# damemi/odigos

Measured on AMD Instinct MI355X. Metric: spans/sec processed (whole node) at 1/2/4/8 MI355X; % of HBM roofline, higher is better.
Workload: dtype u8; 1 GPU; C4: fused odigossampling -> odigosurltemplate -> odigostrafficmetrics, 100M spans in total (all on one GPU at N=1; ~100M/N per GPU, trace-id all-to-all over RCCL at N>1); spans_per_gpu=100000000, spans_total=100000000, template_form=refs, seed=219545604, parallelism=dp1: independent span shards, no data-path collective

## Files before the change

odigos_amd/csrc/engine.cpp:

```cpp
#include <hip/hip_runtime.h>

#include <algorithm>
#include <map>
#include <cstdio>
#include <cstdlib>
#include <cstring>
#include <mutex>
#include <string>
#include <unordered_map>
#include <vector>

#include "../../include/odigos_amd.h"
#include "config.hpp"
#include "devcfg.hpp"
#include "engine_internal.hpp"
#include "kernels.hpp"
#include "slab.hpp"

namespace ose {

thread_local std::string g_last_error;

int fail(int code, const std::string& msg) {
  g_last_error = msg;
  return code;
}

Engine::~Engine() {
  release_exchange_scratch(this);
  release_batch_pool(this);
  release_otlp(this);
  release_encode(this);
  release_condattr(this);
  for (auto& t : timings) { (void)hipEventDestroy(t.a); (void)hipEventDestroy(t.b); }
  for (auto s : streams) (void)hipStreamDestroy(s);
  for (auto ev : event_pool) (void)hipEventDestroy(ev);
  if (url_blob_dev) (void)hipFree(url_blob_dev);
  if (url_blob_forced_dev) (void)hipFree(url_blob_forced_dev);
  for (auto* d : sampling_chunks_dev)
    if (d) (void)hipFree(d);
  for (auto* d : sampling_svc_map_dev)
    if (d) (void)hipFree(d);
  if (sampling_svc_maps_dev) (void)hipFree(sampling_svc_maps_dev);
  if (shard_tables_dev) (void)hipFree(shard_tables_dev);
  if (path_count_dev) (void)hipFree(path_count_dev);
  if (attr_blob_dev) (void)hipFree(attr_blob_dev);
  if (attr_host_mask_dev) (void)hipFree(attr_host_mask_dev);
  for (auto* w : pool) delete w;
}

Workspace::~Workspace() {
  if (dev) (void)hipFree(dev);
  if (table) (void)hipFree(table);
  if (dup_bkt) (void)hipFree(dup_bkt);
  if (dup_bkt_count) (void)hipFree(dup_bkt_count);
  if (runs) (void)hipFree(runs);
  if (run_count) (void)hipFree(run_count);
  if (attr_bits) (void)hipFree(attr_bits);
  if (ep_planes) (void)hipFree(ep_planes);
  if (svc_local) (void)hipFree(svc_local);
  for (void* f : fold)
    if (f) (void)hipFree(f);
  if (dup_host) (void)hipHostFree(dup_host);
  for (hipEvent_t ev : {pending, dup_ready, fork, join, join2})
    if (ev) (void)hipEventDestroy(ev);
}

hipEvent_t Engine::take_event() {
  if (!event_pool.empty()) {
    hipEvent_t ev = event_pool.back();
    event_pool.pop_back();
    return ev;
  }
  hipEvent_t ev = nullptr;
  (void)hipEventCreate(&ev);
  return ev;
}
Engine::Timed Engine::prof_begin(const char* name, hipStream_t st) {
  std::lock_guard<std::mutex> g(mu);
  Timed t{name, take_event(), take_event()};
  (void)hipEventRecord(t.a, st);
  return t;
}
void Engine::prof_end(Timed& t, hipStream_t st) {
  (void)hipEventRecord(t.b, st);
  std::lock_guard<std::mutex> g(mu);
  timings.push_back(t);
}
void Engine::prof_drop(Timed& t) {
  std::lock_guard<std::mutex> g(mu);
  event_pool.push_back(t.a);
  event_pool.push_back(t.b);
}
int Engine::launch_status() {
  HIP_TRY(hipGetLastError());
  return 0;
}

bool stream_capturing(hipStream_t st) {
  hipStreamCaptureStatus cs = hipStreamCaptureStatusNone;
  return hipStreamIsCapturing(st, &cs) == hipSuccess && cs != hipStreamCaptureStatusNone;
}

Workspace* Engine::acquire_ws(hipStream_t st) {
  if (stream_capturing(st)) {
    std::lock_guard<std::mutex> g(mu);
    Workspace* w = nullptr;
    if (!free_ws.empty()) {
      auto it = std::max_element(free_ws.begin(), free_ws.end(),
                                 [](const Workspace* a, const Workspace* b) { return a->cap < b->cap; });
      w = *it;
      free_ws.erase(it);
    } else {
      w = new Workspace();
      pool.push_back(w);
    }
    w->captured = true;
    return w;
  }
  Workspace* w = nullptr;
  {
    std::lock_guard<std::mutex> g(mu);
    if (!free_ws.empty()) {
      w = free_ws.back();
      free_ws.pop_back();
    } else {
      w = new Workspace();
      pool.push_back(w);
    }
  }
  if (w->pending_set) (void)hipStreamWaitEvent(st, w->pending, 0);
  return w;
}
void Engine::return_unused_ws(Workspace* w) {
  std::lock_guard<std::mutex> g(mu);
  w->captured = false;
  free_ws.push_back(w);
}
void Engine::release_ws(Workspace* w, hipStream_t st) {
  if (w->captured) return;
  if (!w->pending) (void)hipEventCreateWithFlags(&w->pending, hipEventDisableTiming);
  w->pending_set = w->pending && hipEventRecord(w->pending, st) == hipSuccess;
  std::lock_guard<std::mutex> g(mu);
  free_ws.push_back(w);
}
#ifndef OSE_SIDE_STREAM_PRIO
#define OSE_SIDE_STREAM_PRIO 0
#endif
hipStream_t Engine::take_stream() {
  std::lock_guard<std::mutex> g(mu);
  if (!free_streams.empty()) {
    hipStream_t s = free_streams.back();
    free_streams.pop_back();
    return s;
  }
  hipStream_t s = nullptr;
#if OSE_SIDE_STREAM_PRIO
  int least = 0, greatest = 0;
  (void)hipDeviceGetStreamPriorityRange(&least, &greatest);
  if (hipStreamCreateWithPriority(&s, hipStreamNonBlocking, greatest) != hipSuccess) return nullptr;
#else
  if (hipStreamCreateWithFlags(&s, hipStreamNonBlocking) != hipSuccess) return nullptr;
#endif
  streams.push_back(s);
  return s;
}
void Engine::give_stream(hipStream_t s) {
  std::lock_guard<std::mutex> g(mu);
  free_streams.push_back(s);
}

int Workspace::reserve(size_t bytes) {
  if (bytes <= cap) return 0;
  if (captured) return fail(OSE_ENOMEM, "workspace too small inside a hipGraph capture: call ose_reserve first");
  if (dev) HIP_TRY(hipFree(dev));
  dev = nullptr;
  cap = 0;
  size_t want = std::max<size_t>(bytes, 1 << 20);
  HIP_TRY(hipMalloc(&dev, want));
  cap = want;
  return 0;
}

int ensure_device() {
  static int status = 1;
  static std::mutex m;
  std::lock_guard<std::mutex> g(m);
  if (status == 1) {
    int n = 0;
    hipError_t e = hipGetDeviceCount(&n);
    status = (e == hipSuccess && n > 0) ? 0 : OSE_EDEVICE;
  }
  if (status) return fail(OSE_EDEVICE, "no HIP device visible: the odigos_amd engine runs only on an MI355X (gfx950)");
  return 0;
}

int bind_device(const Engine* e) {
  int cur = -1;
  if (hipGetDevice(&cur) != hipSuccess || cur != e->device) HIP_TRY(hipSetDevice(e->device));
  return 0;
}

static std::mutex g_dropped_mu;
static uint64_t g_dropped_count = 0;
static std::string g_dropped_last;
void note_dropped_error(const char* where, hipError_t err) {
  std::lock_guard<std::mutex> g(g_dropped_mu);
  g_dropped_count++;
  g_dropped_last = std::string(where) + ": " + hipGetErrorName(err) + " (" + hipGetErrorString(err) + ")";
}

void engine_retain(Engine* e) { e->refs.fetch_add(1, std::memory_order_relaxed); }

void engine_unref(Engine* e) {
  if (e->refs.fetch_sub(1, std::memory_order_acq_rel) != 1) return;
  LastErrorScope keep("engine_unref");
  (void)bind_device(e);
  (void)hipDeviceSynchronize();
  delete e;
}

int upload(const std::vector<uint8_t>& host, uint8_t** dev) {
  HIP_TRY(hipMalloc(dev, host.size()));
  HIP_TRY(hipMemcpy(*dev, host.data(), host.size(), hipMemcpyHostToDevice));
  return 0;
}

int download_columns(const ose_columns& c, const ose_columns* dst) {
  const uint64_t n = c.n_spans, R = c.n_resources, S = c.n_scopes, K = c.n_attr_keys;
  struct F { const void* src; void* dst; size_t bytes; };
  const F fs[] = {
      {c.arena, (void*)dst->arena, c.arena_bytes}, {c.trace_id, (void*)dst->trace_id, 16 * n},
      {c.start_ns, (void*)dst->start_ns, 8 * n}, {c.end_ns, (void*)dst->end_ns, 8 * n},
      {c.status, (void*)dst->status, n}, {c.kind, (void*)dst->kind, n}, {c.resource, (void*)dst->resource, 4 * n},
      {c.scope, (void*)dst->scope, 4 * n}, {c.url_flags, (void*)dst->url_flags, n}, {c.path, (void*)dst->path, 8 * n},
      {c.route, (void*)dst->route, 8 * n}, {c.span_size, (void*)dst->span_size, 4 * n},
      {c.name_len, (void*)dst->name_len, 4 * n},
      {c.attr_match, (void*)dst->attr_match, 8 * n * std::max<uint32_t>(1, c.attr_match_words)},
      {c.res_svc, (void*)dst->res_svc, 4 * R}, {c.res_svc_str, (void*)dst->res_svc_str, 4 * R},
      {c.res_url_ok, (void*)dst->res_url_ok, R}, {c.res_attrset, (void*)dst->res_attrset, 4 * R},
      {c.res_size, (void*)dst->res_size, 4 * R}, {c.scope_size, (void*)dst->scope_size, 4 * S},
      {c.scope_resource, (void*)dst->scope_resource, 4 * S}, {c.attr_type, (void*)dst->attr_type, K * n},
      {c.attr_val, (void*)dst->attr_val, 8 * K * n}, {c.db_flags, (void*)dst->db_flags, n},
      {c.db_query, (void*)dst->db_query, 8 * n}, {c.res_sql_ok, (void*)dst->res_sql_ok, R},
  };
  for (auto& f : fs)
    if (f.src && f.dst && f.bytes) HIP_TRY(hipMemcpy(f.dst, f.src, f.bytes, hipMemcpyDefault));
  return 0;
}

namespace {
int check_stage_mask(const Engine* e, const ose_columns* c, const ose_outputs* o, uint32_t mask) {
  if (mask & OSE_STAGE_CONDATTR) return refuse_condattr("ose_process and ose_process_device");
  if (mask & ~(OSE_STAGE_SAMPLE | OSE_STAGE_TEMPLATE | OSE_STAGE_SIZE | OSE_STAGE_APPLY_KEEP | OSE_STAGE_TEMPLATE_REFS |
               OSE_STAGE_APPLY_TEMPLATE | OSE_STAGE_SQLOP | OSE_STAGE_APPLY_SQLOP))
    return fail(OSE_EINVAL, "unknown stage bit");
  if ((mask & OSE_STAGE_TEMPLATE_REFS) && !(mask & OSE_STAGE_TEMPLATE))
    return fail(OSE_EINVAL, "OSE_STAGE_TEMPLATE_REFS needs OSE_STAGE_TEMPLATE");
  if ((mask & OSE_STAGE_APPLY_KEEP) && (mask & OSE_STAGE_SAMPLE))
    return fail(OSE_EINVAL, "OSE_STAGE_APPLY_KEEP and OSE_STAGE_SAMPLE exclude each other");
  if ((mask & OSE_STAGE_APPLY_TEMPLATE) && (mask & OSE_STAGE_TEMPLATE))
    return fail(OSE_EINVAL, "OSE_STAGE_APPLY_TEMPLATE and OSE_STAGE_TEMPLATE exclude each other");
  if ((mask & OSE_STAGE_APPLY_SQLOP) && (mask & OSE_STAGE_SQLOP))
    return fail(OSE_EINVAL, "OSE_STAGE_APPLY_SQLOP and OSE_STAGE_SQLOP exclude each other");
  if (mask & OSE_STAGE_SQLOP) {
    if (!e->has_sqlop) return fail(OSE_EINVAL, "odigossqldboperationprocessor is not configured on this engine");
    if (!c->db_flags || !c->db_query || !c->resource || !o->sql_op)
      return fail(OSE_EINVAL, "SQLOP stage needs db_flags, db_query, resource and sql_op");
  }
  return 0;
}

struct UrlFork {
  Engine* e;
  Workspace* ws;
  hipStream_t st;
  hipStream_t ust = nullptr;
  bool early_join = false;
  bool join_recorded = false;
  void open() {
    if (!ws->fork) (void)hipEventCreateWithFlags(&ws->fork, hipEventDisableTiming);
    if (!ws->join) (void)hipEventCreateWithFlags(&ws->join, hipEventDisableTiming);
    if (!ws->join2) (void)hipEventCreateWithFlags(&ws->join2, hipEventDisableTiming);
    if (ws->fork && ws->join && ws->join2) ust = e->take_stream();
    if (ust && (hipEventRecord(ws->fork, st) != hipSuccess || hipStreamWaitEvent(ust, ws->fork, 0) != hipSuccess)) {
      e->give_stream(ust);
      ust = nullptr;
    }
  }
  void join(hipEvent_t ev, bool recorded, int& rc) {
    const hipError_t je = recorded ? hipSuccess : hipEventRecord(ev, ust);
    const hipError_t jw = je == hipSuccess ? hipStreamWaitEvent(st, ev, 0) : je;
    if (jw != hipSuccess) {
      (void)hipStreamSynchronize(ust);
      if (!rc) rc = fail(OSE_EDEVICE, std::string("URL stream join: ") + hipGetErrorString(jw));
    }
  }
  void close() {
    if (ust) e->give_stream(ust);
    ust = nullptr;
  }
};

void fuse_size_into_copy(UrlKernelArgs& ua, SizeKernelArgs& sa, Workspace* ws, size_t size_off, const ose_columns* c) {
  sa.kept_partials = size_partials_of(ws, size_off, c->n_scopes, c->n_resources);
  sa.n_kept_partials = url_copy_blocks(ua.n_groups);
  ua.fuse_size = 1;
  ua.size_partials = const_cast<uint32_t*>(sa.kept_partials);
  ua.sz = sa;
}
}

StageOffsets stage_offsets(uint32_t mask, bool defer, uint64_t n, uint64_t n_scopes, uint64_t n_resources,
                           uint64_t arena_bytes, uint32_t url_words) {
  const bool sample = mask & OSE_STAGE_SAMPLE;
  StageOffsets s{};
  s.need = sample ? sampling_scratch_bytes(n) : 0;
  s.url_off = sample ? up(defer ? s.need : 256) : 0;
  s.size_off = sample ? 256 : 0;
  if (mask & OSE_STAGE_TEMPLATE) {
    const size_t url_end = s.url_off + url_workspace_bytes(n, arena_bytes, url_words);
    s.need = std::max(s.need, url_end);
    s.size_off = up(url_end);
  }
  if (mask & OSE_STAGE_SIZE) s.need = std::max(s.need, s.size_off + size_scratch_bytes(n_scopes, n_resources));
  return s;
}

size_t Engine::workspace_bytes(uint64_t n_spans, uint64_t arena_bytes) const {
  const uint32_t mask = (has_sampling ? OSE_STAGE_SAMPLE : 0) | (has_url ? OSE_STAGE_TEMPLATE : 0) |
                        (has_traffic ? OSE_STAGE_SIZE : 0);
  if (has_sampling && has_traffic && !has_url) return sampling_scratch_bytes(n_spans) + size_scratch_bytes(n_spans, n_spans);
  return up(stage_offsets(mask, true, n_spans, n_spans, n_spans, arena_bytes, url_words()).need);
}

int run_stages(Engine* e, const ose_columns* c, const ose_outputs* o, uint32_t mask, uint32_t group_mode,
               const ose_rand* rnd, hipStream_t st) {
  if (!c || !o) return fail(OSE_EINVAL, "columns and outputs are required");
  if (const int mrc = check_stage_mask(e, c, o, mask)) return mrc;
  const bool sql_size = (mask & OSE_STAGE_SIZE) && (mask & (OSE_STAGE_SQLOP | OSE_STAGE_APPLY_SQLOP));
  if (sql_size)
    if (const int src = check_sqlop_size(c, o)) return src;
  const bool capturing = stream_capturing(st);
  if (capturing && (mask & OSE_STAGE_SAMPLE) && group_mode == OSE_GROUP_TRACE_ID)
    return fail(OSE_ENOTSUP, "SAMPLE with OSE_GROUP_TRACE_ID cannot be captured into a hipGraph "
                             "(its trace-id tables advance a host-side generation per call)");
  Workspace* ws = e->acquire_ws(st);
  const uint64_t n = c->n_spans;
  const bool gate_on_host = (mask & OSE_STAGE_SAMPLE) && group_mode == OSE_GROUP_TRACE_ID && n > 0 && !capturing &&
                            !(OSE_DIAG && getenv("OSE_NO_DEFER_SLOW"));
  const bool defer = gate_on_host && (mask & OSE_STAGE_TEMPLATE);
  const StageOffsets so = stage_offsets(mask, defer, n, c->n_scopes, c->n_resources, c->arena_bytes, e->url_words());
  int rc = ws->reserve(so.need);
  const bool tmpl = !rc && (mask & OSE_STAGE_TEMPLATE);
  const bool fused_size_ok = !sql_size && !(OSE_DIAG && getenv("OSE_NO_FUSED_SIZE"));
  std::function<int()> sample_tail;
  UrlKernelArgs ua{};
  UrlFork fork{e, ws, st};
  static const bool one_stream = getenv("OSE_ONE_STREAM") != nullptr;
  constexpr uint64_t kForkSpans = 1u << 20;
  if (!one_stream && !rc && defer && n >= kForkSpans) fork.open();
  ws->beside_url = fork.ust && tmpl;
#ifndef OSE_URL_JOIN_LATE
  fork.early_join = fork.ust && tmpl && (mask & OSE_STAGE_TEMPLATE_REFS) && (mask & OSE_STAGE_SIZE) && fused_size_ok;
#endif
  const uint32_t plan_groups = (uint32_t)((n + kUrlGroup - 1) / kUrlGroup);
  UrlRun ur;
  ur.ws_off = so.url_off;
  ur.refs = (mask & OSE_STAGE_TEMPLATE_REFS) != 0;
  ur.grid_mult = url_plan_grid_mult(plan_groups, fork.ust != nullptr);
  ur.planned = fork.early_join ? ws->join : nullptr;
  if (fork.ust && tmpl) {
    rc = run_url(e, c, o, fork.ust, ws, ur, &ua);
    fork.join_recorded = fork.early_join && !rc;
  }
  if (!rc && (mask & OSE_STAGE_SAMPLE)) rc = run_sampling(e, c, o, group_mode, rnd, st, ws, gate_on_host ? &sample_tail : nullptr);
  if (sample_tail && !defer) {
    rc = sample_tail();
    sample_tail = nullptr;
  }
  if (!fork.ust && tmpl && !rc) rc = run_url(e, c, o, st, ws, ur, &ua);
  if (sample_tail) {
    const int trc = sample_tail();
    if (!rc) rc = trc;
  }
  if (fork.ust) fork.join(ws->join, fork.join_recorded, rc);
  if (!rc && (mask & OSE_STAGE_SQLOP)) rc = run_sqlop(e, c, o, st);
  SizeKernelArgs sa{};
  bool size_on = false;
  if (!rc && (mask & OSE_STAGE_SIZE)) rc = prepare_size(e, c, o, mask, group_mode, rnd, st, ws, so.size_off, sa, size_on);
  if (!rc && tmpl) {
    if (size_on && n > 0 && fused_size_ok) fuse_size_into_copy(ua, sa, ws, so.size_off, c);
    rc = run_url_back(e, ua, st);
  }
  if (!rc && size_on) rc = sql_size ? run_sqlop_size_tail(e, sa, o->sql_op, st) : run_size_tail(e, sa, st);
  if (fork.join_recorded) fork.join(ws->join2, false, rc);
  fork.close();
  ws->beside_url = false;
  e->release_ws(ws, st);
  return rc;
}

}

using namespace ose;

extern "C" {

const char* ose_last_error(void) { return g_last_error.c_str(); }

uint64_t ose_dropped_errors(char* last, size_t cap) {
  std::lock_guard<std::mutex> g(g_dropped_mu);
  if (last && cap) snprintf(last, cap, "%s", g_dropped_last.c_str());
  return g_dropped_count;
}

extern "C" void osehost_stage_offsets(uint32_t mask, int defer, uint64_t n_spans, uint64_t n_scopes, uint64_t n_resources,
                                      uint64_t arena_bytes, uint32_t url_words, uint64_t* out) {
  const StageOffsets so = stage_offsets(mask, defer != 0, n_spans, n_scopes, n_resources, arena_bytes, url_words);
  Engine e;
  e.has_sampling = mask & OSE_STAGE_SAMPLE;
  e.has_url = mask & OSE_STAGE_TEMPLATE;
  e.has_traffic = mask & OSE_STAGE_SIZE;
  e.url_nfa_words = url_words;
  out[0] = so.url_off;
  out[1] = so.size_off;
  out[2] = so.need;
  out[3] = e.workspace_bytes(n_spans, arena_bytes);
}

int ose_engine_create(const char* cfg_json, ose_engine** out) {
  if (!out) return fail(OSE_EINVAL, "out is NULL");
  *out = nullptr;
  Json root;
  try {
    root = parse_json(cfg_json ? cfg_json : "{}");
  } catch (const std::exception& ex) {
    return fail(OSE_EINVAL, ex.what());
  }
  if (!root.is_obj()) return fail(OSE_EINVAL, "config must be a JSON object");
  auto* e = new Engine();
  std::string err;
  if (const Json* j = root.get("odigosurltemplate")) {
    err = decode_url_config(*j, e->url);
    if (!err.empty()) { delete e; return fail(OSE_EINVAL, err); }
    e->has_url = true;
    e->url_needs_resource = e->url.include.has_value() || e->url.exclude.has_value();
  }
  if (const Json* j = root.get("odigossampling")) {
    err = decode_sampling_config(*j, e->sampling);
    if (!err.empty()) { delete e; return fail(OSE_EINVAL, err); }
    e->has_sampling = true;
  }
  if (const Json* j = root.get("odigostrafficmetrics")) {
    err = decode_traffic_config(*j, e->traffic);
    if (!err.empty()) { delete e; return fail(OSE_EINVAL, err); }
    e->has_traffic = true;
    e->inverse = e->traffic.sampling_ratio != 0 ? (int64_t)(1.0 / e->traffic.sampling_ratio) : 0;
  }
  if (const Json* j = root.get("odigossqldboperationprocessor")) {
    err = decode_sqlop_config(*j, e->sqlop);
    if (!err.empty()) { delete e; return fail(OSE_EINVAL, err); }
    e->has_sqlop = true;
  }
  if (const Json* j = root.get("odigosconditionalattributes")) {
    err = decode_condattr_config(*j, e->condattr);
    if (!err.empty()) { delete e; return fail(OSE_EINVAL, err); }
    if (const int crc = compile_condattr(e->condattr, e->condattr_tab)) { delete e; return crc; }
    e->has_condattr = true;
  }
  if (e->has_url) {
    int rc = build_url_blob(e->url, e->url_blob_host, e->max_name, false, e->url_nfa_words);
    if (rc) { delete e; return rc; }
  }
  int rc = e->build_sampling_tables();
  if (rc) { delete e; return rc; }
  rc = e->build_attr_tables();
  if (rc) { delete e; return rc; }
  rc = ensure_device();
  if (rc) { delete e; return rc; }
  if (hipGetDevice(&e->device) != hipSuccess) { delete e; return fail(OSE_EDEVICE, "hipGetDevice failed"); }
  if (e->has_url) {
    rc = upload(e->url_blob_host, &e->url_blob_dev);
    if (rc) { delete e; return rc; }
  }
  rc = e->upload_sampling_tables();
  if (rc) { delete e; return rc; }
  if (e->has_condattr) {
    rc = upload(e->condattr_tab.blob, &e->condattr_blob_dev);
    if (rc) { delete e; return rc; }
  }
  if (!e->attr_blob_host.empty()) {
    rc = upload(e->attr_blob_host, &e->attr_blob_dev);
    if (rc) { delete e; return rc; }
    std::vector<uint8_t> hm(8 * std::max<size_t>(e->attr_words, 1), 0);
    std::memcpy(hm.data(), e->attr_host_words.data(), 8 * std::min<size_t>(e->attr_host_words.size(), e->attr_words));
    rc = upload(hm, &e->attr_host_mask_dev);
    if (rc) { delete e; return rc; }
  }
  {
    hipError_t he = hipMalloc(reinterpret_cast<void**>(&e->path_count_dev), 64);
    if (he == hipSuccess) he = hipMemset(e->path_count_dev, 0, 64);
    if (he != hipSuccess) {
      delete e;
      return fail(OSE_EDEVICE, std::string("path counters: ") + hipGetErrorString(he));
    }
  }
  *out = reinterpret_cast<ose_engine*>(e);
  return 0;
}

uint32_t ose_engine_path_counts(ose_engine* eng, uint64_t* counts, uint32_t cap) {
  if (!eng) return 0;
  Engine* e = reinterpret_cast<Engine*>(eng);
  uint64_t c[5] = {0, 0, 0, 0, 0};
  if (e->path_count_dev && bind_device(e) == 0) {
    LastErrorScope keep("ose_engine_path_counts");
    if (hipDeviceSynchronize() != hipSuccess ||
        hipMemcpy(c, e->path_count_dev, 32, hipMemcpyDeviceToHost) != hipSuccess)
      c[0] = c[1] = c[2] = c[3] = 0;
  }
  c[4] = c[3];
  c[3] = c[2];
  c[2] = e->long_run_passes.load();
  for (uint32_t k = 0; k < 5 && k < cap && counts; k++) counts[k] = c[k];
  return 5;
}

uint64_t ose_engine_url_nfa_groups(ose_engine* eng) {
  if (!eng) return 0;
  Engine* e = reinterpret_cast<Engine*>(eng);
  uint64_t c = 0;
  if (e->path_count_dev && bind_device(e) == 0) {
    LastErrorScope keep("ose_engine_url_nfa_groups");
    if (hipDeviceSynchronize() != hipSuccess || hipMemcpy(&c, e->path_count_dev + 4, 8, hipMemcpyDeviceToHost) != hipSuccess)
      c = 0;
  }
  return c;
}

void ose_engine_destroy(ose_engine* eng) {
  if (!eng) return;
  Engine* e = reinterpret_cast<Engine*>(eng);
  e->closed.store(true);
  engine_unref(e);
}

int ose_host_alloc(size_t bytes, void** out) {
  if (!out) return fail(OSE_EINVAL, "NULL argument");
  int rc = ensure_device();
  if (rc) return rc;
  HIP_TRY(hipHostMalloc(out, bytes ? bytes : 1, hipHostMallocDefault));
  return 0;
}
void ose_host_free(void* p) {
  LastErrorScope keep("ose_host_free");
  if (p) (void)hipHostFree(p);
}

int ose_set_device(int device) {
  int rc = ensure_device();
  if (rc) return rc;
  HIP_TRY(hipSetDevice(device));
  return 0;
}

uint32_t ose_engine_service_id(const ose_engine* eng, const char* name, size_t len) {
  if (!eng || !name) return OSE_NONE;
  const Engine* e = reinterpret_cast<const Engine*>(eng);
  auto it = e->service_ids.find(std::string(name, len));
  return it == e->service_ids.end() ? OSE_NONE : it->second;
}

int ose_engine_get_info(const ose_engine* eng, ose_engine_info* info) {
  if (!eng || !info) return fail(OSE_EINVAL, "NULL argument");
  const Engine* e = reinterpret_cast<const Engine*>(eng);
  info->stages = (e->has_sampling ? OSE_STAGE_SAMPLE : 0) | (e->has_url ? OSE_STAGE_TEMPLATE : 0) |
                 (e->has_traffic ? OSE_STAGE_SIZE : 0) | (e->has_sqlop ? OSE_STAGE_SQLOP : 0) |
                 (e->has_condattr ? OSE_STAGE_CONDATTR : 0);
  info->max_template_name = e->max_name;
  info->inverse_sampling = e->inverse;
  info->traffic_sampling_ratio = e->traffic.sampling_ratio;
  info->n_attr_rules = e->attr_n_rules;
  info->n_attr_keys = (uint32_t)e->attr_keys.size();
  info->attr_host_rules = e->attr_host_rules;
  return 0;
}

uint32_t ose_engine_attr_host_rules(const ose_engine* eng, uint64_t* words, uint32_t cap) {
  if (!eng) return 0;
  const Engine* e = reinterpret_cast<const Engine*>(eng);
  if (!e->attr_n_rules) return 0;
  const uint32_t W = e->attr_words;
  for (uint32_t w = 0; w < W && w < cap && words; w++) words[w] = w < e->attr_host_words.size() ? e->attr_host_words[w] : 0;
  return W;
}

int ose_engine_set_option(ose_engine* eng, const char* name, int64_t value) {
  if (!eng || !name) return fail(OSE_EINVAL, "NULL argument");
  Engine* e = reinterpret_cast<Engine*>(eng);
  static const struct { const char* name; uint32_t bit; } kOpts[] = {
      {"otlp_gpu_chain", Engine::kOptOtlpGpuChain},
      {"otlp_host_resources", Engine::kOptOtlpHostResources},
      {"otlp_host_scopes", Engine::kOptOtlpHostScopes},
      {"encode_host", Engine::kOptEncodeHost},
      {"otlp_sqlop", Engine::kOptOtlpSqlop},
      {"url_path_counts", Engine::kOptUrlPathCounts},
      {"otlp_condattr", Engine::kOptOtlpCondattr},
      {"url_regex_nfa", Engine::kOptUrlRegexNfa},
  };
  for (const auto& o : kOpts) {
    if (strcmp(name, o.name) != 0) continue;
    if (o.bit == Engine::kOptOtlpSqlop && !e->has_sqlop)
      return fail(OSE_EINVAL, "engine option otlp_sqlop: odigossqldboperationprocessor is not configured");
    if (o.bit == Engine::kOptOtlpCondattr) {
      if (!e->has_condattr)
        return fail(OSE_EINVAL, "engine option otlp_condattr: odigosconditionalattributes is not configured");
      if (value)
        if (const int rc = build_condattr_keytab(e)) return rc;
    }
    if (o.bit == Engine::kOptUrlRegexNfa) {
      if (!e->has_url) return fail(OSE_EINVAL, "engine option url_regex_nfa: odigosurltemplate is not configured");
      if (value && !e->url_blob_forced_dev) {
        if (int brc = bind_device(e)) return brc;
        std::vector<uint8_t> blob;
        uint32_t max_name = 0, words = 0;
        if (const int rc = build_url_blob(e->url, blob, max_name, true, words)) return rc;
        if (const int rc = upload(blob, &e->url_blob_forced_dev)) return rc;
        e->url_forced_words = words;
      }
    }
    if (value) e->options.fetch_or(o.bit);
    else e->options.fetch_and(~o.bit);
    return 0;
  }
  return fail(OSE_EINVAL, std::string("unknown engine option: ") + name);
}

int ose_reserve(ose_engine* eng, uint64_t n_spans, uint64_t arena_bytes) {
  if (!eng) return fail(OSE_EINVAL, "NULL engine");
  Engine* e = reinterpret_cast<Engine*>(eng);
  if (int brc = bind_device(e)) return brc;
  Workspace* ws = e->acquire_ws(nullptr);
  int rc = ws->reserve(e->workspace_bytes(n_spans, arena_bytes));
  if (!rc && e->has_sampling) rc = ws->reserve_table(n_spans);
  if (!rc && e->attr_n_dev) rc = ws->reserve_attr(n_spans);
  if (!rc && e->sampling_chunks_dev.size() > 1) rc = ws->reserve_fold(std::max<uint64_t>(n_spans, 1));
  e->release_ws(ws, nullptr);
  return rc;
}

int ose_process_device(ose_engine* eng, const ose_columns* cols, const ose_outputs* outs, uint32_t stage_mask,
                       uint32_t group_mode, const ose_rand* rnd, void* hip_stream) {
  if (!eng) return fail(OSE_EINVAL, "NULL engine");
  if (int brc = bind_device(reinterpret_cast<Engine*>(eng))) return brc;
  return run_stages(reinterpret_cast<Engine*>(eng), cols, outs, stage_mask, group_mode, rnd,
                    static_cast<hipStream_t>(hip_stream));
}

int ose_profile_enable(ose_engine* eng, int on) {
  if (!eng) return fail(OSE_EINVAL, "NULL engine");
  reinterpret_cast<Engine*>(eng)->profiling = on != 0;
  return 0;
}

int ose_profile_read(ose_engine* eng, char* json, size_t cap) {
  if (!eng || !json) return fail(OSE_EINVAL, "NULL argument");
  Engine* e = reinterpret_cast<Engine*>(eng);
  if (int brc = bind_device(e)) return brc;
  std::vector<Engine::Timed> ts;
  {
    std::lock_guard<std::mutex> g(e->mu);
    ts.swap(e->timings);
  }
  std::map<std::string, std::pair<uint64_t, double>> acc;
  for (auto& t : ts) {
    HIP_TRY(hipEventSynchronize(t.b));
    float ms = 0;
    HIP_TRY(hipEventElapsedTime(&ms, t.a, t.b));
    auto& a = acc[t.name];
    a.first++;
    a.second += ms;
  }
  {
    std::lock_guard<std::mutex> g(e->mu);
    for (auto& t : ts) { e->event_pool.push_back(t.a); e->event_pool.push_back(t.b); }
  }
  std::string s = "{";
  for (auto& kv : acc) {
    if (s.size() > 1) s += ",";
    char buf[256];
    snprintf(buf, sizeof buf, "\"%s\":{\"launches\":%llu,\"ms\":%.6f}", kv.first.c_str(),
             (unsigned long long)kv.second.first, kv.second.second);
    s += buf;
  }
  s += "}";
  if (s.size() + 1 > cap) return fail(OSE_ERANGE, "profile buffer too small");
  std::memcpy(json, s.c_str(), s.size() + 1);
  return 0;
}

int ose_device_info(char* buf, size_t cap) {
  if (!buf || cap == 0) return fail(OSE_EINVAL, "NULL buffer");
  int rc = ensure_device();
  if (rc) { snprintf(buf, cap, "no device"); return rc; }
  hipDeviceProp_t p;
  HIP_TRY(hipGetDeviceProperties(&p, 0));
  snprintf(buf, cap, "%s arch=%s CUs=%d HBM=%.1fGB", p.name, p.gcnArchName, p.multiProcessorCount,
           (double)p.totalGlobalMem / 1e9);
  return 0;
}

}
```

odigos_amd/csrc/engine_internal.hpp:

```cpp
#pragma once
#include <hip/hip_runtime.h>

#include <atomic>
#include <cstdint>
#include <functional>
#include <mutex>
#include <string>
#include <unordered_map>
#include <vector>

#include "../../include/odigos_amd.h"
#include "config.hpp"
#include "condattr_host.hpp"
#include "slab.hpp"
#include "timed_launch.hpp"

namespace ose {

int fail(int code, const std::string& msg);
#define HIP_TRY(expr)                                                                                  \
  do {                                                                                                 \
    hipError_t _e = (expr);                                                                            \
    if (_e != hipSuccess) return fail(OSE_EDEVICE, std::string(#expr) + ": " + hipGetErrorString(_e)); \
  } while (0)
struct Engine;
int bind_device(const Engine* e);
int upload(const std::vector<uint8_t>& host, uint8_t** dev);
int ensure_device();
void engine_retain(Engine* e);
void engine_unref(Engine* e);
void note_dropped_error(const char* where, hipError_t err);
struct LastErrorScope {
  const char* where;
  hipError_t prev;
  explicit LastErrorScope(const char* w) : where(w), prev(hipPeekAtLastError()) {}
  ~LastErrorScope() {
    if (prev != hipSuccess) return;
    const hipError_t now = hipGetLastError();
    if (now != hipSuccess) note_dropped_error(where, now);
  }
};
bool stream_capturing(hipStream_t st);
struct Engine;
void release_exchange_scratch(const Engine* e);
void release_batch_pool(Engine* e);
struct OtlpEngine;
void release_otlp(Engine* e);
void release_encode(Engine* e);
void release_condattr(Engine* e);
int build_condattr_keytab(Engine* e);

struct OtlpBatchView {
  Engine* e;
  const ose_columns* cols;
  bool released;
  const uint64_t* d_spans;
  bool res_on_device;
  const uint64_t *d_res_ref, *d_scope_ref;
  const uint64_t *h_res_ref, *h_scope_ref;
  size_t h_res_n, h_scope_n;
};
void otlp_batch_view(const ose_otlp_batch* b, OtlpBatchView* v);
struct OtlpReleasedLayout {
  const uint64_t* spans;
  const uint32_t* span0;
  const uint64_t *hdr, *schema;
  const uint64_t* res_ref;
  const uint32_t* res_scope0;
  const uint64_t* scope_ref;
};
ose_otlp_batch* otlp_released_new(Engine* e);
void otlp_released_delete(ose_otlp_batch* b);
int otlp_released_arena(ose_otlp_batch* b, size_t bytes, uint8_t** p);
void otlp_released_set(ose_otlp_batch* b, const ose_columns& cols, const OtlpReleasedLayout& lay);

struct Workspace {
  void* dev = nullptr;
  size_t cap = 0;
  hipEvent_t pending = nullptr;
  bool pending_set = false;
  bool captured = false;
  int reserve(size_t bytes);
  void* table = nullptr;
  uint64_t table_slots_cap = 0;
  uint64_t* dup_bkt = nullptr;
  uint32_t* dup_bkt_count = nullptr;
  uint32_t dup_bkt_bits = 0;
  uint32_t epoch = 0;
  int reserve_table(uint64_t n_spans);
  uint32_t* runs = nullptr;
  uint32_t* run_count = nullptr;
  uint64_t runs_slots = 0;
  int reserve_runs();
  void* fold[2] = {nullptr, nullptr};
  uint64_t fold_cap = 0;
  int reserve_fold(uint64_t n_spans);
  uint64_t* attr_bits = nullptr;
  uint64_t attr_bits_cap = 0;
  int reserve_attr(uint64_t n_spans);
  uint64_t* ep_planes = nullptr;
  uint64_t ep_planes_cap = 0;
  ose_columns spill_cols{};
  uint32_t* svc_local = nullptr;
  uint64_t svc_local_cap = 0;
  ose_columns local_cols{};
  int reserve_svc_local(uint64_t n_resources);
  int reserve_ep_planes(uint64_t words);
  uint32_t* dup_host = nullptr;
  hipEvent_t dup_ready = nullptr;
  hipEvent_t fork = nullptr, join = nullptr, join2 = nullptr;
  bool beside_url = false;
  Workspace() = default;
  Workspace(const Workspace&) = delete;
  ~Workspace();
};

struct Engine {
  std::atomic<int> refs{1};
  std::atomic<bool> closed{false};
  int device = 0;
  UrlTemplateConfig url;
  SamplingConfig sampling;
  TrafficMetricsConfig traffic;
  SqlOpConfig sqlop;
  bool has_url = false, has_sampling = false, has_traffic = false, has_sqlop = false;
  CondAttrConfig condattr;
  bool has_condattr = false;
  CondAttrCompiled condattr_tab;
  uint8_t* condattr_blob_dev = nullptr;
  std::mutex condattr_mu;
  void* condattr_pin = nullptr;
  void* condattr_stage = nullptr;
  size_t condattr_pin_cap = 0, condattr_stage_cap = 0;
  void* condattr_slots_dev = nullptr;
  uint32_t condattr_slot_mask = 0;
  uint64_t condattr_key_lens = 0;
  enum : uint32_t {
    kOptOtlpGpuChain = 1, kOptOtlpHostResources = 2, kOptOtlpHostScopes = 4, kOptEncodeHost = 8, kOptOtlpSqlop = 16,
    kOptUrlPathCounts = 32,
    kOptOtlpCondattr = 64,
    kOptUrlRegexNfa = 128
  };
  std::atomic<uint32_t> options{0};
  bool option(uint32_t o) const { return (options.load(std::memory_order_relaxed) & o) != 0; }
  bool url_needs_resource = false;
  int64_t inverse = 1;
  uint32_t max_name = 5;

  std::vector<uint8_t> url_blob_host;
  uint8_t* url_blob_dev = nullptr;
  uint32_t url_nfa_words = 0;
  uint8_t* url_blob_forced_dev = nullptr;
  uint32_t url_forced_words = 0;
  bool url_forced() const { return option(kOptUrlRegexNfa) && url_blob_forced_dev; }
  uint32_t url_words() const { return url_forced() ? url_forced_words : url_nfa_words; }
  std::vector<uint8_t> sampling_blob_host;
  uint8_t* sampling_blob_dev = nullptr;
  std::vector<std::vector<uint8_t>> sampling_chunks_host;
  std::vector<uint8_t*> sampling_chunks_dev;
  std::vector<uint8_t> sampling_chunk_attr;
  std::vector<uint32_t> sampling_lat_svc;
  uint8_t* shard_tables_dev = nullptr;
  unsigned long long* path_count_dev = nullptr;
  std::atomic<uint64_t> long_run_passes{0};
  std::unordered_map<std::string, uint32_t> service_ids;
  uint32_t sampling_n_lat = 0, sampling_n_attr = 0;
  uint32_t sampling_n_lat_svc = 0;
  bool sampling_walk_ok = false;
  bool sampling_spill = false;
  bool sampling_local_svc = false;
  std::vector<std::vector<uint32_t>> sampling_svc_map_host;
  std::vector<uint32_t*> sampling_svc_map_dev;
  uint32_t** sampling_svc_maps_dev = nullptr;
  std::vector<uint8_t> attr_blob_host;
  uint8_t* attr_blob_dev = nullptr;
  uint32_t attr_n_rules = 0, attr_n_dev = 0;
  uint64_t attr_host_rules = 0;
  std::vector<uint64_t> attr_host_words;
  uint32_t attr_words = 1;
  uint8_t* attr_host_mask_dev = nullptr;
  bool attr_host_rules_any() const {
    for (uint64_t w : attr_host_words)
      if (w) return true;
    return false;
  }
  std::vector<std::string> attr_keys;

  std::mutex mu;
  std::vector<Workspace*> pool, free_ws;
  std::vector<void*> batch_pool;
  OtlpEngine* otlp = nullptr;
  std::vector<void*> otlp_pool;
  std::vector<void*> enc_pool;
  size_t batch_pool_bytes = 0;

  bool profiling = false;
  struct Timed { const char* name; hipEvent_t a, b; };
  std::vector<Timed> timings;
  std::vector<hipEvent_t> event_pool;
  template <class F>
  int timed(const char* name, hipStream_t st, F&& launch) {
    return timed_launch(*this, name, st, std::forward<F>(launch));
  }

 private:
  template <class P, class S, class F>
  friend int timed_launch(P& p, const char* name, S st, F&& launch);
  hipEvent_t take_event();
  Timed prof_begin(const char* name, hipStream_t st);
  void prof_end(Timed& t, hipStream_t st);
  void prof_drop(Timed& t);
  int launch_status();

 public:

  ~Engine();
  Workspace* acquire_ws(hipStream_t st);
  void release_ws(Workspace* w, hipStream_t st);
  void return_unused_ws(Workspace* w);
  std::vector<hipStream_t> streams, free_streams;
  hipStream_t take_stream();
  void give_stream(hipStream_t s);
  int build_sampling_tables();
  int upload_sampling_tables();
  int build_attr_tables();
  size_t workspace_bytes(uint64_t n_spans, uint64_t arena_bytes) const;
};

int run_sampling(Engine* e, const ose_columns* c, const ose_outputs* o, uint32_t group_mode, const ose_rand* rnd,
                 hipStream_t st, Workspace* ws, std::function<int()>* tail = nullptr);
struct SamplingLayout {
  WsPart win_heads, win_base, wstatus, rec, key, k2, v2, k3, v3, hist, hoff, hstatus, long_runs, long_meta, long_pieces,
      long_part, win_first;
  size_t end;
};
SamplingLayout sampling_layout(uint64_t n_spans);
template <class L>
uint32_t layout_parts(const L& l, uint64_t* off, uint64_t* bytes, uint32_t cap, uint64_t* end) {
  constexpr uint32_t kParts = (sizeof(L) - sizeof(size_t)) / sizeof(WsPart);
  static_assert(sizeof(L) == kParts * sizeof(WsPart) + sizeof(size_t), "WsParts, then end");
  const WsPart* p = reinterpret_cast<const WsPart*>(&l);
  for (uint32_t k = 0; k < kParts && k < cap; k++) {
    if (off) off[k] = p[k].off;
    if (bytes) bytes[k] = p[k].bytes;
  }
  if (end) *end = l.end;
  return kParts;
}
size_t sampling_scratch_bytes(uint64_t n_spans);
struct TraceSortArgs;
int radix_passes(TraceSortArgs s, uint32_t* const kb[2], uint32_t* const vb[2], uint32_t* hist, uint32_t* hoff,
                 uint32_t htiles, int bits, const uint32_t* keys_in, const uint32_t* vals_in, hipStream_t st,
                 const uint32_t** keys, const uint32_t** vals);
int download_columns(const ose_columns& src, const ose_columns* dst);
int resolve_attr_match(Engine* e, const ose_columns* c, Workspace* ws, hipStream_t st, const uint64_t** out);
int run_size(Engine* e, const ose_columns* c, const ose_outputs* o, uint32_t mask, uint32_t group_mode,
             const ose_rand* rnd, hipStream_t st, Workspace* ws, size_t off);
struct SizeKernelArgs;
int prepare_size(Engine* e, const ose_columns* c, const ose_outputs* o, uint32_t mask, uint32_t group_mode,
                 const ose_rand* rnd, hipStream_t st, Workspace* ws, size_t off, SizeKernelArgs& a, bool& active);
uint32_t* size_partials_of(Workspace* ws, size_t off, uint64_t n_scopes, uint64_t n_resources);
int run_size_tail(Engine* e, const SizeKernelArgs& a, hipStream_t st);
int run_size_scopes(Engine* e, const SizeKernelArgs& a, hipStream_t st);
size_t size_scratch_bytes(uint64_t n_scopes, uint64_t n_resources);
int run_sqlop(Engine* e, const ose_columns* c, const ose_outputs* o, hipStream_t st);
int check_sqlop_size(const ose_columns* c, const ose_outputs* o);
int run_sqlop_size_tail(Engine* e, const SizeKernelArgs& a, const uint8_t* sql_op, hipStream_t st);
int refuse_condattr(const char* entry);
int spill_endpoint_planes(Engine* e, const ose_columns* c, Workspace* ws, hipStream_t st, const uint64_t** out);
struct StageOffsets { size_t url_off, size_off, need; };
StageOffsets stage_offsets(uint32_t mask, bool defer, uint64_t n_spans, uint64_t n_scopes, uint64_t n_resources,
                           uint64_t arena_bytes, uint32_t url_words);
int run_stages(Engine* e, const ose_columns* c, const ose_outputs* o, uint32_t mask, uint32_t group_mode,
               const ose_rand* rnd, hipStream_t st);
int build_url_blob(const UrlTemplateConfig& c, std::vector<uint8_t>& out, uint32_t& max_name, bool force_nfa,
                   uint32_t& nfa_words);
struct UrlLayout {
  WsPart zero, bump, slow_aligned, scan_status;
  WsPart len, meta, code, gsum, gbase, gscr, slow, unpl, dbg;
  WsPart scr;
  WsPart slab;
  size_t end;
};
UrlLayout url_layout(uint64_t n_spans, uint64_t arena_bytes, uint32_t nfa_words, bool refs);
size_t url_workspace_bytes(uint64_t n_spans, uint64_t arena_bytes, uint32_t nfa_words = 0);
struct UrlKernelArgs;
struct UrlRun {
  size_t ws_off = 0;
  bool refs = false;
  uint32_t grid_mult = 1;
  hipEvent_t planned = nullptr;
};
int run_url(Engine* e, const ose_columns* c, const ose_outputs* o, hipStream_t st, Workspace* ws, const UrlRun& r,
            UrlKernelArgs* front);
int run_url_back(Engine* e, const UrlKernelArgs& a, hipStream_t st);

}
```

odigos_amd/csrc/kernels.hpp:

```cpp
#pragma once
#include <hip/hip_runtime.h>

#include <cstdint>

#include "../../include/odigos_amd.h"

#ifndef OSE_DIAG
#define OSE_DIAG 0
#endif

namespace ose {

struct SizePart {
  uint32_t r;
  uint32_t ch;
  uint64_t v;
};
struct SizeKernelArgs {
  uint64_t n_spans;
  uint32_t n_scopes, n_resources, n_attrsets;
  uint32_t sampled;
  uint32_t templated;
  uint32_t remove_empty;
  const uint32_t* batch_keep;
  const uint32_t* span_size;
  const uint32_t* name_len;
  const uint32_t* scope;
  const uint32_t* scope_size;
  const uint32_t* scope_resource;
  const uint32_t* res_size;
  const uint32_t* res_attrset;
  const uint8_t* keep;
  const uint8_t* url_out;
  const uint8_t* kind;
  const ose_strref* tmpl;
  int64_t inverse;
  uint64_t* scope_body;
  SizePart* parts;
  uint32_t* fix;
  uint32_t n_swin;
  int64_t* attrset_bytes;
  int64_t* accepted;
  uint64_t* res_bytes;
  const uint32_t* kept_partials;
  uint32_t n_kept_partials;
};

struct UrlKernelArgs {
  uint64_t n_spans;
  uint32_t n_groups;
  const uint8_t* arena;
  const uint8_t* url_flags;
  const uint8_t* kind;
  const uint32_t* resource;
  const uint8_t* res_url_ok;
  const ose_strref* path;
  uint8_t* url_out;
  ose_strref* tmpl;
  uint8_t* out_arena;
  uint64_t out_cap;
  const uint8_t* cfg;
  uint32_t* plan_len;
  uint32_t* plan_meta;
  uint64_t* plan_code;
  uint8_t* scratch;
  uint64_t scr_region;
  uint64_t* group_scr;
  uint64_t* group_sum;
  uint64_t* group_base;
  uint32_t n_scan_tiles;
  uint32_t* scan_counter;
  uint64_t* scan_status;
  uint32_t* error;
  uint64_t* used;
  uint32_t* slow_count;
  uint32_t* slow_groups;
  uint32_t* unplanned_count;
  uint32_t* unplanned;
  uint32_t general;
  uint32_t nfa, nfa_words;
  uint32_t* nfa_slab;
  uint32_t refs;
  uint64_t* bump;
  uint64_t refs_chunk;
  uint32_t plan_waves;
  uint64_t* slow_aligned;
  uint32_t plan_grid_mult;
  uint32_t ablate;
  uint64_t* dbg;
  uint32_t fuse_size;
  uint32_t* size_partials;
  SizeKernelArgs sz;
};
constexpr uint32_t kUrlCopyMaxBlocks = 65536;
uint32_t url_copy_blocks(uint32_t n_groups);
constexpr uint32_t kUrlGroup = 64;
constexpr uint32_t kUrlScanTile = 1024;
constexpr uint32_t kUrlMaxWaves = 4096;
constexpr uint32_t kUrlWaveSlack = 8192;
inline size_t url_scratch_bytes(uint64_t n, uint64_t arena_bytes) {
  const uint64_t g = (n + kUrlGroup - 1) / kUrlGroup;
  const uint64_t w = g < kUrlMaxWaves ? g : kUrlMaxWaves;
  return ((arena_bytes + n + (arena_bytes + n) / 4 + 15) & ~15ull) + w * kUrlWaveSlack;
}
constexpr uint32_t kUrlNfaMaxWaves = 1024;
inline uint32_t url_nfa_waves(uint64_t n) {
  const uint64_t g = ((n + kUrlGroup - 1) / kUrlGroup + 3) & ~3ull;
  return (uint32_t)(g < kUrlNfaMaxWaves ? g : kUrlNfaMaxWaves);
}
inline size_t url_nfa_slab_bytes(uint64_t n, uint32_t nfa_words) {
  return nfa_words ? 256 + (size_t)url_nfa_waves(n) * 2 * nfa_words * kUrlGroup * 4 : 0;
}
#ifndef OSE_PLAN_GRID_OLD
#define OSE_PLAN_GRID_OLD 0
#endif
inline uint32_t url_plan_grid_mult(uint32_t n_groups, bool forked = false) {
  if (OSE_PLAN_GRID_OLD) return forked ? 16u : 1u;
  const uint32_t m = n_groups / (kUrlMaxWaves * 19u);
  return m < 1 ? 1u : m > 16 ? 16u : m;
}
void launch_url_plan(const UrlKernelArgs& a, hipStream_t st);
uint32_t url_plan_waves(const UrlKernelArgs& a);
uint64_t url_refs_chunk(uint64_t cap, uint32_t waves);
void launch_url_scan(const UrlKernelArgs& a, hipStream_t st);
void launch_url_copy(const UrlKernelArgs& a, hipStream_t st);
void launch_url_plan_slow(const UrlKernelArgs& a, hipStream_t st);
void launch_url_emit_slow(const UrlKernelArgs& a, hipStream_t st);
void launch_url_nfa_fill(const UrlKernelArgs& a, hipStream_t st);
void launch_url_nfa_plan(const UrlKernelArgs& a, hipStream_t st);
void launch_url_nfa_emit(const UrlKernelArgs& a, hipStream_t st);

}

namespace ose {

struct TraceSlot {
  uint32_t state;
  uint32_t first;
  uint64_t hi, lo;
  uint64_t _pad;
};
struct TraceRec {
  uint32_t first_span;
  uint8_t keep, level, _p0, _p1;
  double ratio;
};
enum : uint32_t { kTraceRuns = 0, kTracePerm = 1, kTraceBatch = 2 };
struct FoldState {
  double ratio;
  double min_fb;
  uint32_t level;
  uint32_t flags;
};
enum : uint32_t { kFsSat = 1, kFsMatched = 2, kFsFoundFb = 4, kFsHaveMin = 8, kFsDone = 16 };
struct SampWalkDev;
struct TraceKernelArgs {
  uint64_t n_spans;
  uint32_t n_windows;
  uint32_t mode;
  uint32_t n_resources;
  uint32_t epoch;
  const FoldState* fold_in;
  FoldState* fold_out;
  const uint64_t* tid;
  const uint64_t* start;
  const uint64_t* end;
  const uint8_t* status;
  const uint32_t* resource;
  const ose_strref* route;
  const uint8_t* arena;
  const uint32_t* res_svc;
  const uint32_t* res_svc_str;
  const uint8_t* cfg;
  uint64_t seed;
  uint8_t* keep;
  TraceRec* rec;
  uint64_t* win_heads;
  TraceSlot* table;
  uint64_t table_mask;
  uint32_t* dup;
  uint32_t* dup_bkt_count;
  uint64_t* dup_bkt;
  uint32_t dup_bkt_bits;
  const uint32_t* perm;
  const uint32_t* key;
  uint32_t* error;
  uint32_t* batch_keep;
  const uint64_t* route_match;
  const uint64_t* attr_match;
  uint64_t attr_stride;
  uint32_t attr_words;
  const uint64_t* svc_match;
  uint32_t ablate;
  uint32_t* n_long;
  uint32_t* long_runs;
  uint4* long_meta;
  uint2* long_pieces;
  uint8_t* long_part;
  uint32_t long_steps;
  uint32_t win_per_wave;
  uint32_t narrow;
  const uint8_t* const* cfgs;
  uint32_t n_multi;
  uint32_t cfg_lds_bytes;
  const uint32_t* lat_gslot;
  const SampWalkDev* walks;
  uint32_t* run_count;
  uint32_t* runs;
  uint32_t* overflow;
  unsigned long long* path_count;
  uint64_t* win_first;
  uint32_t* head_slot;
};
constexpr uint32_t kMaxRuns = 8;
constexpr uint32_t kMaxFoldSpans = 4096;
constexpr uint32_t kMaxFoldSlots = 8;
#ifndef OSE_WPW_BESIDE
#define OSE_WPW_BESIDE 64
#endif
constexpr uint32_t kWinPerWaveBeside = OSE_WPW_BESIDE;
constexpr uint32_t kWinPerWave = 16;
#ifndef OSE_LONG_PIECE
#define OSE_LONG_PIECE 2048
#endif
constexpr uint32_t kLongPiece = OSE_LONG_PIECE;
constexpr uint32_t kLongPartBytes = 1344;
inline uint64_t long_piece_cap(uint64_t n) { return n / 64 + 1 + n / kLongPiece + 1; }
inline uint64_t long_part_cap(uint64_t n) { return 2 * (n / kLongPiece) + 2; }
constexpr uint32_t kLongSteps = 4;
void launch_trace_eval(const TraceKernelArgs& a, hipStream_t st);
constexpr uint32_t kMaxMulti = 3;
constexpr uint32_t kMultiCfgLds = 24576;
constexpr uint32_t kDupBucketCap = 1024;
void launch_trace_dup_check(const TraceKernelArgs& a, hipStream_t st);
void launch_trace_long(const TraceKernelArgs& a, hipStream_t st, uint32_t known_runs = 0);
void launch_trace_insert_exact(const TraceKernelArgs& a, hipStream_t st);
void launch_trace_runs(const TraceKernelArgs& a, hipStream_t st);
void launch_trace_fold(const TraceKernelArgs& a, hipStream_t st);
void launch_trace_first_select(const TraceKernelArgs& a, hipStream_t st);

struct TraceSortArgs {
  uint64_t n_spans;
  uint32_t n_tiles;
  uint32_t shift;
  const uint32_t* gate;
  const uint64_t* tid;
  const TraceSlot* table;
  uint64_t table_mask;
  uint32_t epoch;
  const uint32_t* keys_in;
  const uint32_t* vals_in;
  uint32_t* keys_out;
  uint32_t* vals_out;
  uint32_t* hist;
  uint32_t* key;
  uint32_t* error;
  unsigned long long* path_count;
  uint32_t* scan_counter;
  uint64_t* scan_status;
  uint32_t scan_status_n;
};
constexpr uint32_t kSortTile = 4096;
void launch_trace_key(const TraceSortArgs& a, hipStream_t st);
void launch_sort_hist(const TraceSortArgs& a, hipStream_t st);
void launch_sort_scatter(const TraceSortArgs& a, hipStream_t st);

struct ScanArgs {
  uint64_t n;
  uint32_t n_tiles;
  uint32_t popcount;
  const uint32_t* gate;
  const void* in;
  uint32_t* out;
  uint32_t* total;
  uint32_t* counter;
  uint64_t* status;
  uint32_t* error;
};
constexpr uint32_t kScanTileItems = 1024;
void launch_scan_u32(const ScanArgs& a, hipStream_t st);

struct TraceCompactArgs {
  uint32_t n_windows;
  const uint64_t* win_heads;
  const uint32_t* win_base;
  const TraceRec* rec;
  uint32_t* trace_first_span;
  uint8_t* trace_keep;
  uint8_t* trace_level;
  double* trace_ratio;
};
void launch_trace_compact(const TraceCompactArgs& a, hipStream_t st);

struct ShardArgs {
  uint64_t n_spans;
  uint32_t n_tiles;
  uint32_t n_ranks;
  const uint64_t* tid;
  const uint64_t* start;
  const uint64_t* end;
  const uint8_t* status;
  const uint32_t* resource;
  const ose_strref* route;
  const uint8_t* arena;
  const uint64_t* route_match;
  uint64_t rm_stride;
  const uint64_t* attr_match;
  uint64_t attr_stride;
  uint32_t attr_words;
  const uint32_t* res_svc;
  const uint32_t* res_svc_str;
  const uint8_t* const* cfgs;
  uint32_t n_chunks;
  const uint32_t* lat_svc;
  uint32_t n_global_svc;
  const uint32_t* const* svc_maps;
  uint32_t cfg_lds_bytes;
  uint32_t* hist;
  uint32_t* hoff;
  uint64_t* counts;
  uint8_t* send;
  uint32_t* pack_pos;
};
constexpr uint32_t kXSteps = 16;
constexpr uint32_t kXChunk = kXSteps * 64;
constexpr uint32_t kXFixedWords = 5;
constexpr uint32_t kXRecBytes = 8 * (kXFixedWords + 2);
constexpr uint32_t x_rec_words(uint32_t n_chunks) { return kXFixedWords + 2 * n_chunks; }
constexpr uint32_t x_rec_bytes(uint32_t n_chunks) { return 8 * x_rec_words(n_chunks); }
void launch_shard_hist(const ShardArgs& a, hipStream_t st);
void launch_shard_counts(const ShardArgs& a, hipStream_t st);
void launch_shard_scatter(const ShardArgs& a, hipStream_t st);
struct UnpackArgs {
  const uint8_t* recv;
  uint64_t n;
  uint32_t n_chunks;
  uint64_t* tid;
  uint64_t* start;
  uint64_t* end;
  uint8_t* status;
  uint32_t* resource;
  uint32_t* res_svc;
  uint32_t* res_svc_str;
  uint64_t* route_match;
  uint64_t* svc_match;
};
void launch_shard_unpack(const UnpackArgs& a, hipStream_t st);
constexpr uint32_t kOwnerCap = 256;
constexpr uint32_t kOwnerAvg = 80;
constexpr uint32_t kOwnerSlotWords = 8;
struct OwnerArgs {
  const uint8_t* recv;
  uint64_t n;
  uint32_t words;
  uint32_t n_buckets;
  uint32_t* bkt_count;
  uint64_t* bkt_rec;
  const uint8_t* const* cfgs;
  uint32_t n_chunks;
  const uint32_t* const* svc_maps;
  uint32_t n_global_svc;
  uint32_t cfg_lds_bytes;
  uint64_t seed;
  uint8_t* keep;
  uint32_t* overflow;
  uint64_t* clocks;
};
void launch_owner_bucket(const OwnerArgs& a, hipStream_t st);
void launch_owner_fold(const OwnerArgs& a, hipStream_t st);
void launch_scatter_keep(const uint8_t* back, const uint32_t* pos, uint64_t n, uint8_t* keep, hipStream_t st);
void launch_svc_translate(const uint32_t* map, uint32_t n_global, const uint32_t* in1, const uint32_t* in2, uint32_t* out1,
                          uint32_t* out2, uint64_t n, hipStream_t st);
void launch_endpoint_plane(const uint8_t* cfg, const uint32_t* resource, const uint32_t* res_svc, const ose_strref* route,
                           const uint8_t* arena, uint64_t n, uint64_t* out, hipStream_t st);
struct PeerCopies {
  const uint8_t* src[64];
  uint8_t* dst[64];
  uint64_t len[64];
  uint32_t n;
};
void launch_peer_copies(const PeerCopies& c, uint64_t max_len, hipStream_t st);
void launch_add_i64(int64_t* dst, const int64_t* src, uint64_t n, hipStream_t st);
uint32_t shard_owner_host(uint64_t hi, uint64_t lo, uint32_t n_ranks);

constexpr uint32_t kBatchKeepWord = 16;

void launch_size_spans(const SizeKernelArgs& a, hipStream_t st);
void launch_size_tail(const SizeKernelArgs& a, hipStream_t st);
void launch_size_fix(const SizeKernelArgs& a, hipStream_t st);

struct SqlOpArgs {
  uint64_t n_spans;
  const uint8_t* arena;
  const uint8_t* db_flags;
  const ose_strref* db_query;
  const uint32_t* resource;
  const uint8_t* res_sql_ok;
  uint8_t* sql_op;
};
void launch_sqlop(const SqlOpArgs& a, hipStream_t st);
struct SqlSizeArgs {
  SizeKernelArgs sz;
  const uint8_t* sql_op;
};
void launch_sqlop_size_spans(const SqlSizeArgs& a, hipStream_t st);

struct CondAttrArgs {
  const uint8_t* blob;
  ose_condattr_columns c;
  ose_condattr_outputs o;
};
void launch_condattr_scopes(const CondAttrArgs& a, hipStream_t st);
void launch_condattr_spans(const CondAttrArgs& a, hipStream_t st);

struct AttrArgs {
  uint64_t n_spans;
  const uint8_t* type;
  const uint64_t* val;
  const uint8_t* arena;
  const uint32_t* resource;
  const uint32_t* res_svc;
  uint32_t words;
  const uint64_t* host_bits;
// ... 419 lines not shown
```

odigos_amd/csrc/size_host.cpp:

```cpp
#include <algorithm>

#include "engine_internal.hpp"
#include "kernels.hpp"
#include "slab.hpp"

namespace ose {

namespace {
struct SizeLayout {
  size_t scope, parts, fix, partials, end;
};
SizeLayout size_layout(uint64_t n_scopes) {
  const uint64_t W = (std::max<uint64_t>(n_scopes, 1) + 63) / 64;
  SizeLayout L;
  L.scope = 256;
  L.parts = up(L.scope + 8 * std::max<uint64_t>(n_scopes, 1));
  L.fix = up(L.parts + 32 * W);
  L.partials = up(L.fix + 4 * W);
  L.end = up(L.partials + 4ull * kUrlCopyMaxBlocks) + 256;
  return L;
}
}
size_t size_scratch_bytes(uint64_t n_scopes, uint64_t n_resources) {
  (void)n_resources;
  return size_layout(n_scopes).end;
}

int prepare_size(Engine* e, const ose_columns* c, const ose_outputs* o, uint32_t mask, uint32_t group_mode,
                 const ose_rand* rnd, hipStream_t st, Workspace* ws, size_t off, SizeKernelArgs& a, bool& active) {
  active = false;
  if (!e->has_traffic) return fail(OSE_EINVAL, "odigostrafficmetrics is not configured on this engine");
  if (!o->attrset_bytes || !o->accepted_spans) return fail(OSE_EINVAL, "SIZE stage needs attrset_bytes and accepted_spans");
  const uint64_t n = c->n_spans;
  if (n && (!c->span_size || !c->scope)) return fail(OSE_EINVAL, "SIZE stage needs span_size and scope");
  if (c->n_scopes && (!c->scope_size || !c->scope_resource)) return fail(OSE_EINVAL, "SIZE stage needs scope_size and scope_resource");
  if (c->n_resources && (!c->res_size || !c->res_attrset)) return fail(OSE_EINVAL, "SIZE stage needs res_size and res_attrset");
  const bool applied = mask & OSE_STAGE_APPLY_KEEP;
  const bool sampled = (mask & OSE_STAGE_SAMPLE) || applied;
  const bool templated = mask & (OSE_STAGE_TEMPLATE | OSE_STAGE_APPLY_TEMPLATE);
  if (applied && n && !o->keep) return fail(OSE_EINVAL, "OSE_STAGE_APPLY_KEEP needs keep");
  if (templated && n && (!c->kind || !c->name_len || !o->url_out || !o->tmpl))
    return fail(OSE_EINVAL, "SIZE after TEMPLATE needs kind, name_len, url_out and tmpl");
  const double ratio = e->traffic.sampling_ratio;
  const double u = rnd ? rnd->traffic_u : 0.0;
  if (!(ratio != 0 && u < ratio)) return 0;
  const uint64_t S = c->n_scopes, R = c->n_resources;
  int rc = ws->reserve(off + size_scratch_bytes(S, R));
  if (rc) return rc;
  uint8_t* base = static_cast<uint8_t*>(ws->dev) + off;
  const SizeLayout L = size_layout(S);
  uint8_t* sc = base + L.scope;
  HIP_TRY(hipMemsetAsync(sc, 0, 8 * std::max<uint64_t>(S, 1), st));
  a = SizeKernelArgs{};
  a.n_spans = n;
  a.n_scopes = (uint32_t)S;
  a.n_resources = (uint32_t)R;
  a.n_attrsets = c->n_attrsets;
  a.sampled = sampled;
  a.templated = templated;
  a.remove_empty = applied || (sampled && group_mode == OSE_GROUP_TRACE_ID);
  a.batch_keep = !applied && sampled && group_mode == OSE_GROUP_BATCH
                     ? reinterpret_cast<const uint32_t*>(ws->dev) + kBatchKeepWord : nullptr;
  a.span_size = c->span_size;
  a.name_len = c->name_len;
  a.scope = c->scope;
  a.scope_size = c->scope_size;
  a.scope_resource = c->scope_resource;
  a.res_size = c->res_size;
  a.res_attrset = c->res_attrset;
  a.keep = o->keep;
  a.url_out = o->url_out;
  a.kind = c->kind;
  a.tmpl = o->tmpl;
  a.inverse = e->inverse;
  a.scope_body = reinterpret_cast<uint64_t*>(sc);
  a.parts = reinterpret_cast<SizePart*>(base + L.parts);
  a.fix = reinterpret_cast<uint32_t*>(base + L.fix);
  a.n_swin = (uint32_t)((S + 63) / 64);
  a.attrset_bytes = o->attrset_bytes;
  a.accepted = o->accepted_spans;
  a.res_bytes = o->res_bytes;
  a.kept_partials = nullptr;
  a.n_kept_partials = 0;
  active = true;
  return 0;
}

uint32_t* size_partials_of(Workspace* ws, size_t off, uint64_t n_scopes, uint64_t n_resources) {
  (void)n_resources;
  return reinterpret_cast<uint32_t*>(static_cast<uint8_t*>(ws->dev) + off + size_layout(n_scopes).partials);
}

int run_size_tail(Engine* e, const SizeKernelArgs& a, hipStream_t st) {
  if (!a.kept_partials)
    if (const int rc = e->timed("size_span_kernel", st, [&] { launch_size_spans(a, st); })) return rc;
  return run_size_scopes(e, a, st);
}
int run_size_scopes(Engine* e, const SizeKernelArgs& a, hipStream_t st) {
  if (const int rc = e->timed("size_tail_kernel", st, [&] { launch_size_tail(a, st); })) return rc;
  return e->timed("size_fix_kernel", st, [&] { launch_size_fix(a, st); });
}

int run_size(Engine* e, const ose_columns* c, const ose_outputs* o, uint32_t mask, uint32_t group_mode,
             const ose_rand* rnd, hipStream_t st, Workspace* ws, size_t off) {
  SizeKernelArgs a;
  bool active = false;
  int rc = prepare_size(e, c, o, mask, group_mode, rnd, st, ws, off, a, active);
  if (rc || !active) return rc;
  return run_size_tail(e, a, st);
}

}
```

odigos_amd/csrc/url_host.cpp:

```cpp
#include <hip/hip_runtime.h>

#include <algorithm>
#include <cstdio>
#include <cstdlib>
#include <cstring>
#include <string>
#include <vector>

#include "../../include/odigos_amd.h"
#include "blob.hpp"
#include "config.hpp"
#include "devcfg.hpp"
#include "engine_internal.hpp"
#include "kernels.hpp"
#include "regex_dfa.hpp"
#include "regex_nfa.hpp"
#include "slab.hpp"

namespace ose {

int build_url_blob(const UrlTemplateConfig& c, std::vector<uint8_t>& out, uint32_t& max_name, bool force_nfa,
                   uint32_t& nfa_words) {
  Blob bl;
  UrlCfgDev h{};
  bl.put(&h, 1);
  std::string bytes;
  std::vector<NameDev> names;
  auto add_text = [&](const std::string& s) {
    NameDev n{(uint32_t)bytes.size(), (uint32_t)s.size()};
    bytes += s;
    return n;
  };
  names.push_back(add_text("id"));
  names.push_back(add_text("date"));
  names.push_back(add_text("email"));
  std::vector<Dfa> dfas;
  std::vector<std::vector<uint8_t>> nfas;
  nfa_words = 0;
  auto compile = [&](const std::string& rx, int32_t& idx) -> int {
    Dfa d;
    std::string err;
    RegexStatus st = force_nfa ? RegexStatus::TooLarge : compile_dfa(rx, d, err);
    if (st == RegexStatus::Ok) {
      idx = (int32_t)dfas.size();
      dfas.push_back(std::move(d));
      return 0;
    }
    if (st == RegexStatus::TooLarge) {
      NfaProgram np;
      err.clear();
      st = compile_nfa(rx, np, err);
      if (st == RegexStatus::Ok) {
        idx = url_nfa_code((uint32_t)nfas.size());
        nfa_words = std::max(nfa_words, np.words());
        nfas.push_back(nfa_image(np));
        return 0;
      }
    }
    if (st == RegexStatus::Syntax) return fail(OSE_EINVAL, err);
    return fail(OSE_ENOTSUP, "regexp not supported by the DFA and NFA compilers: " + err);
  };
  std::vector<UrlCustomDev> custom;
  for (auto& ci : c.custom_ids) {
    UrlCustomDev cd{};
    int rc = compile(ci.regexp, cd.dfa);
    if (rc) return rc;
    cd.name = (uint32_t)names.size();
    names.push_back(add_text(ci.template_name.empty() ? "id" : ci.template_name));
    custom.push_back(cd);
  }
  struct ParsedRule { uint32_t nseg; size_t order; std::vector<RuleSegment> segs; };
  std::vector<ParsedRule> rules;
  for (size_t k = 0; k < c.templatization_rules.size(); k++) {
    ParsedRule pr;
    std::string e = parse_user_rule(c.templatization_rules[k], pr.segs);
    if (!e.empty()) return fail(OSE_EINVAL, e);
    pr.nseg = (uint32_t)pr.segs.size();
    pr.order = k;
    rules.push_back(std::move(pr));
  }
  std::stable_sort(rules.begin(), rules.end(), [](const ParsedRule& a, const ParsedRule& b) { return a.nseg < b.nseg; });
  uint32_t longest = 0;
  for (auto& r : rules) longest = std::max(longest, r.nseg);
  std::vector<uint32_t> by_len(longest + 2, 0);
  std::vector<UrlRuleDev> rdev;
  std::vector<UrlRuleSegDev> sdev;
  uint32_t max_nseg = 0;
  for (auto& r : rules) {
    rdev.push_back(UrlRuleDev{r.nseg, (uint32_t)sdev.size()});
    max_nseg = std::max(max_nseg, r.nseg);
    for (auto& s : r.segs) {
      UrlRuleSegDev sd{};
      sd.dfa = -1;
      switch (s.kind) {
        case SegKind::Static: sd.kind = kRuleStatic; break;
        case SegKind::Wildcard: sd.kind = kRuleWildcard; break;
        case SegKind::Template: sd.kind = kRuleTemplate; break;
        case SegKind::Regex: sd.kind = kRuleRegex; break;
      }
      NameDev t = add_text(s.text);
      sd.text_off = t.off;
      sd.text_len = t.len;
      if (s.has_regexp) {
        int rc = compile(s.regexp, sd.dfa);
        if (rc) return rc;
      }
      sdev.push_back(sd);
    }
  }
  for (uint32_t n = 0; n <= longest + 1; n++) {
    uint32_t k = 0;
    while (k < rules.size() && rules[k].nseg < n) k++;
    by_len[n] = k;
  }
  max_name = 0;
  for (auto& n : names) max_name = std::max(max_name, n.len);
  h.n_custom = (uint32_t)custom.size();
  h.n_rules = (uint32_t)rdev.size();
  h.n_names = (uint32_t)names.size();
  h.n_dfa = (uint32_t)dfas.size();
  h.max_rule_nseg = max_nseg;
  h.max_name_len = max_name;
  h.rules_by_len_off = bl.put(by_len.data(), by_len.size());
  h.rules_off = bl.put(rdev.data(), rdev.size());
  h.segs_off = bl.put(sdev.data(), sdev.size());
  h.custom_off = bl.put(custom.data(), custom.size());
  h.names_off = bl.put(names.data(), names.size());
  std::vector<uint32_t> dfa_offs;
  for (auto& d : dfas) dfa_offs.push_back(put_dfa(bl, d));
  h.dfa_off = bl.put(dfa_offs.data(), dfa_offs.size());
  h.bytes_off = bl.put(bytes.data(), bytes.size());
  if (!nfas.empty()) {
    std::vector<uint32_t> nfa_offs;
    for (auto& im : nfas) nfa_offs.push_back(bl.put(im.data(), im.size()));
    h.n_nfa = (uint32_t)nfas.size();
    h.nfa_off = bl.put(nfa_offs.data(), nfa_offs.size());
  }
  bl.align();
  if (bl.overflow)
    return fail(OSE_ENOTSUP, "odigosurltemplate device tables exceed 4 GiB (the regexps' DFAs and NFA programs together)");
  bl.b.resize(bl.b.size() + 16, 0);
  h.total_bytes = (uint32_t)bl.b.size();
  std::memcpy(bl.b.data(), &h, sizeof h);
  out = std::move(bl.b);
  return 0;
}

UrlLayout url_layout(uint64_t n, uint64_t arena_bytes, uint32_t nfa_words, bool refs) {
  const size_t g = (n + kUrlGroup - 1) / kUrlGroup;
  const size_t t = (g + kUrlScanTile - 1) / kUrlScanTile;
  Carve c;
  auto part = [&](size_t bytes, size_t align = 256) { return WsPart{c.take(bytes, align), bytes}; };
  UrlLayout L;
  L.zero = part(32 + 8 * t);
  L.bump = {16, 8};
  L.slow_aligned = {24, 8};
  L.scan_status = {32, 8 * t};
  L.len = part(4 * n);
  L.meta = part(4 * n, 4);
  L.code = part(8 * n, 8);
  L.gsum = part(8 * g, 8);
  L.gbase = part(8 * g, 8);
  L.gscr = part(8 * g, 8);
  L.slow = part(4 * g, 4);
  L.unpl = part(4 * g, 4);
  L.dbg = part(256);
  L.scr = part(refs ? 0 : url_scratch_bytes(n, arena_bytes));
  L.slab = nfa_words ? part(url_nfa_slab_bytes(n, nfa_words) - 256) : WsPart{c.off, 0};
  L.end = c.off;
  return L;
}

size_t url_workspace_bytes(uint64_t n, uint64_t arena_bytes, uint32_t nfa_words) {
  return url_layout(n, arena_bytes, nfa_words, false).end;
}

namespace {
UrlKernelArgs url_args(const Engine* e, const ose_columns* c, const ose_outputs* o, uint8_t* base, const UrlLayout& L,
                       const UrlRun& r) {
  auto at = [&](const WsPart& p) { return base + p.off; };
  const uint64_t n = c->n_spans;
  const uint32_t nfa_words = e->url_words();
  UrlKernelArgs a{};
  a.n_spans = n;
  a.n_groups = (uint32_t)((n + kUrlGroup - 1) / kUrlGroup);
  a.arena = c->arena;
  a.url_flags = c->url_flags;
  a.kind = c->kind;
  a.resource = c->resource;
  a.res_url_ok = c->res_url_ok;
  a.path = c->path;
  a.url_out = o->url_out;
  a.tmpl = o->tmpl;
  a.out_arena = o->tmpl_arena;
  a.out_cap = o->tmpl_arena_cap;
  a.cfg = e->url_forced() ? e->url_blob_forced_dev : e->url_blob_dev;
  a.nfa = nfa_words ? 1u : 0u;
  a.nfa_words = nfa_words;
  a.nfa_slab = nfa_words ? reinterpret_cast<uint32_t*>(at(L.slab)) : nullptr;
  a.general = (!e->url.custom_ids.empty() || !e->url.templatization_rules.empty()) ? 1u : 0u;
  a.plan_len = reinterpret_cast<uint32_t*>(at(L.len));
  a.plan_meta = reinterpret_cast<uint32_t*>(at(L.meta));
  a.plan_code = reinterpret_cast<uint64_t*>(at(L.code));
  a.group_sum = reinterpret_cast<uint64_t*>(at(L.gsum));
  a.group_base = reinterpret_cast<uint64_t*>(at(L.gbase));
  a.group_scr = reinterpret_cast<uint64_t*>(at(L.gscr));
  a.scratch = at(L.scr);
  if (r.refs) {
    a.refs = 1;
    a.scratch = o->tmpl_arena;
    a.bump = reinterpret_cast<uint64_t*>(at(L.bump));
    a.slow_aligned = reinterpret_cast<uint64_t*>(at(L.slow_aligned));
  }
  a.n_scan_tiles = (uint32_t)(L.scan_status.bytes / 8);
  a.scan_counter = reinterpret_cast<uint32_t*>(base);
  a.scan_status = reinterpret_cast<uint64_t*>(at(L.scan_status));
  a.error = o->device_status ? o->device_status : reinterpret_cast<uint32_t*>(base + 8);
  a.slow_count = reinterpret_cast<uint32_t*>(base + 4);
  a.slow_groups = reinterpret_cast<uint32_t*>(at(L.slow));
  a.unplanned_count = reinterpret_cast<uint32_t*>(base + 12);
  a.unplanned = reinterpret_cast<uint32_t*>(at(L.unpl));
  a.used = o->tmpl_arena_used;
#if OSE_DIAG
  if (const char* ab = getenv("OSE_URL_ABLATE")) a.ablate = (uint32_t)strtoul(ab, nullptr, 0);
#endif
  a.plan_grid_mult = r.refs ? r.grid_mult : 1u;
  a.scr_region = (url_scratch_bytes(n, c->arena_bytes) / std::max<uint32_t>(1, url_plan_waves(a))) & ~15ull;
  a.plan_waves = url_plan_waves(a);
  a.refs_chunk = url_refs_chunk(o->tmpl_arena_cap, a.plan_waves);
  return a;
}

int queue_url_front(Engine* e, const UrlKernelArgs& a, hipStream_t st, hipEvent_t planned) {
  int rc;
  if (a.nfa) {
    if ((rc = e->timed("url_nfa_fill_kernel", st, [&] { launch_url_nfa_fill(a, st); }))) return rc;
    if ((rc = e->timed("url_nfa_plan_kernel", st, [&] { launch_url_nfa_plan(a, st); }))) return rc;
  } else {
    if ((rc = e->timed("url_plan_kernel", st, [&] { launch_url_plan(a, st); }))) return rc;
    if ((rc = e->timed("url_plan_slow_kernel", st, [&] { launch_url_plan_slow(a, st); }))) return rc;
  }
  if (planned) HIP_TRY(hipEventRecord(planned, st));
  if ((rc = e->timed("url_scan_kernel", st, [&] { launch_url_scan(a, st); }))) return rc;
  rc = e->timed(a.nfa ? "url_nfa_emit_kernel" : "url_emit_slow_kernel", st, [&] {
    if (a.nfa) launch_url_nfa_emit(a, st);
    else launch_url_emit_slow(a, st);
  });
  if (rc) return rc;
  if ((e->options.load() & Engine::kOptUrlPathCounts) && e->path_count_dev) {
    HIP_TRY(hipMemcpyAsync(e->path_count_dev + 2, a.unplanned_count, 4, hipMemcpyDeviceToDevice, st));
    HIP_TRY(hipMemcpyAsync(e->path_count_dev + 3, a.slow_count, 4, hipMemcpyDeviceToDevice, st));
    if (a.nfa) HIP_TRY(hipMemcpyAsync(e->path_count_dev + 4, a.unplanned_count, 4, hipMemcpyDeviceToDevice, st));
    else HIP_TRY(hipMemsetAsync(e->path_count_dev + 4, 0, 8, st));
  }
  return 0;
}

int print_url_clocks(const UrlKernelArgs& a, hipStream_t st) {
  uint64_t h[16];
  uint32_t cnt[4];
  HIP_TRY(hipMemcpyAsync(h, a.dbg, sizeof h, hipMemcpyDeviceToHost, st));
  HIP_TRY(hipMemcpyAsync(cnt, a.scan_counter, sizeof cnt, hipMemcpyDeviceToHost, st));
  HIP_TRY(hipStreamSynchronize(st));
  const double wp = h[3] ? (double)h[3] : 1.0;
  fprintf(stderr, "url clocks/wave: plan[stage %.0f bitmaps %.0f plan %.0f assemble+store %.0f]\n", h[0] / wp,
          h[1] / wp, h[2] / wp, h[5] / wp);
  fprintf(stderr, "url plan list clocks/wave: enumerate %.0f classify %.0f fold %.0f\n", h[13] / wp, h[14] / wp,
          h[15] / wp);
  fprintf(stderr, "url groups: %llu, slow (K3s) %u, unplanned (K1b) %u\n", (unsigned long long)((a.n_spans + 63) / 64),
          cnt[1], cnt[3]);
  fprintf(stderr, "url_plan_slow_kernel slowest block clocks: config %llu whole %llu plan_path %llu\n",
          (unsigned long long)h[8], (unsigned long long)h[9], (unsigned long long)h[10]);
  return 0;
}
}

int run_url(Engine* e, const ose_columns* c, const ose_outputs* o, hipStream_t st, Workspace* ws, const UrlRun& r,
            UrlKernelArgs* front) {
  if (!e->has_url) return fail(OSE_EINVAL, "odigosurltemplate is not configured on this engine");
  if (!c->url_flags || !c->kind || !c->path || !c->arena || !o->url_out || !o->tmpl || !o->tmpl_arena)
    return fail(OSE_EINVAL, "TEMPLATE stage needs url_flags, kind, path, arena, url_out, tmpl, tmpl_arena");
  if (e->url_needs_resource && (!c->resource || !c->res_url_ok))
    return fail(OSE_EINVAL, "include/exclude configured: resource and res_url_ok columns are required");
  if (c->res_url_ok && !c->resource) return fail(OSE_EINVAL, "res_url_ok needs the resource column");
  if (o->tmpl_arena_cap > 0xFFFFFFFFull) return fail(OSE_ERANGE, "tmpl_arena_cap exceeds the 32-bit offset range");
  const UrlLayout L = url_layout(c->n_spans, c->arena_bytes, e->url_words(), r.refs);
  int rc = ws->reserve(r.ws_off + L.end);
  if (rc) return rc;
  uint8_t* base = static_cast<uint8_t*>(ws->dev) + r.ws_off;
  HIP_TRY(hipMemsetAsync(base, 0, L.zero.bytes, st));
  UrlKernelArgs a = url_args(e, c, o, base, L, r);
  *front = a;
  if (a.n_spans == 0) {
    if (o->tmpl_arena_used) HIP_TRY(hipMemsetAsync(o->tmpl_arena_used, 0, 8, st));
    if (r.planned) HIP_TRY(hipEventRecord(r.planned, st));
    return 0;
  }
  if (a.ablate & 512) {
    a.dbg = reinterpret_cast<uint64_t*>(base + L.dbg.off);
    HIP_TRY(hipMemsetAsync(a.dbg, 0, 256, st));
  }
  rc = queue_url_front(e, a, st, r.planned);
  if (!rc) *front = a;
  return rc;
}

int run_url_back(Engine* e, const UrlKernelArgs& a, hipStream_t st) {
  if (a.n_spans == 0) return 0;
  if (!a.refs || a.fuse_size)
    if (const int rc = e->timed("url_copy_kernel", st, [&] { launch_url_copy(a, st); })) return rc;
  return (a.ablate & 512) ? print_url_clocks(a, st) : 0;
}

}

using namespace ose;

extern "C" uint32_t osehost_url_layout(uint64_t n_spans, uint64_t arena_bytes, uint32_t nfa_words, int refs, uint64_t* off,
                                       uint64_t* bytes, uint32_t cap, uint64_t* end, uint64_t* workspace_bytes) {
  if (workspace_bytes) *workspace_bytes = url_workspace_bytes(n_spans, arena_bytes, nfa_words);
  return layout_parts(url_layout(n_spans, arena_bytes, nfa_words, refs != 0), off, bytes, cap, end);
}

extern "C" int osehost_url_blob_hash(const char* cfg_json, int force_nfa, uint64_t* hash, uint64_t* bytes,
                                     uint32_t* n_nfa) {
  Json root;
  try {
    root = parse_json(cfg_json ? cfg_json : "{}");
  } catch (const std::exception& ex) {
    return fail(OSE_EINVAL, ex.what());
  }
  const Json* j = root.is_obj() ? root.get("odigosurltemplate") : nullptr;
  if (!j) return fail(OSE_EINVAL, "odigosurltemplate is not configured");
  UrlTemplateConfig url;
  const std::string err = decode_url_config(*j, url);
  if (!err.empty()) return fail(OSE_EINVAL, err);
  std::vector<uint8_t> blob;
  uint32_t max_name = 0, words = 0;
  if (const int rc = build_url_blob(url, blob, max_name, force_nfa != 0, words)) return rc;
  uint64_t h = 0xcbf29ce484222325ull;
  for (uint8_t b : blob) h = (h ^ b) * 0x100000001b3ull;
  if (hash) *hash = h;
  if (bytes) *bytes = blob.size();
  if (n_nfa) *n_nfa = reinterpret_cast<const UrlCfgDev*>(blob.data())->n_nfa;
  return 0;
}
```

odigos_amd/csrc/url_kernel.hip:

```cpp
#include <hip/hip_runtime.h>

#include <algorithm>
#include <cstdlib>

#include "../../include/odigos_amd.h"
#include "device_common.hpp"
#include "kernels.hpp"
#include "regex_nfa_device.hpp"
#include "size_device.hpp"
#include "url_classes.hpp"

#ifndef OSE_ASM_BATCH
#define OSE_ASM_BATCH 0
#endif

namespace ose {
namespace {

constexpr int kThreads = 256;
constexpr int kWaves = kThreads / kWave;
constexpr uint32_t kStage = 4 * 1024;

enum : uint32_t { M_NONE = 0, M_RENAME_SLASH, M_SLASH, M_RULE, M_DEFAULT, M_ORIG };

// ... 972 lines not shown
    const uint32_t r = a >> 5, sh = a & 31;
    k += __builtin_popcount(__builtin_amdgcn_alignbit(b32[4 * kRowVec * (r + 1) + c], b32[4 * kRowVec * r + c], sh) &
                            (uint32_t)low_mask(e - a));
    a += 32;
  }
  return k;
}

__device__ __forceinline__ uint64_t half_mask(uint32_t lo, uint32_t hi, uint32_t base) {
  const uint32_t l = lo > base ? min(lo - base, 64u) : 0u, h = hi > base ? min(hi - base, 64u) : 0u;
  return low_mask(h) & ~low_mask(l);
}

__device__ __noinline__ uint32_t name_len_global(const uint8_t* blob, uint32_t names_off, uint32_t id) {
  return reinterpret_cast<const NameDev*>(blob + names_off)[id].len;
}
__device__ __forceinline__ uint32_t name_len(const Cfg& cfg, uint32_t id) {
  if (cfg.names_tab_all || id < kNameTab) return cfg.name_tab[id].len;
  return name_len_global(cfg.blob, cfg.names_off, id);
}


__device__ __forceinline__ bool plan_group_list(const Cfg& cfg, lds_u32* stage32, lds_cu4* bm, uint32_t* segs,
                                                bool needs_path, uint32_t p0, uint32_t plen, uint32_t f, Plan& p,
                                                bool tm, uint64_t* tt, uint32_t* cls = nullptr,
                                                uint32_t* seg_off = nullptr, bool* big_id = nullptr) {
  if (!cls) cls = segs;
  const int lane = threadIdx.x & 63;
  uint64_t c0 = tm ? clk() : 0;
  LdsReader rd(stage32, p0);
  const lds_u32* b32 = (const lds_u32*)bm;
  uint32_t n = 0, nseg = 0;
  const uint32_t r0 = p0 >> 5, b0 = p0 & 31;
  const bool win = needs_path && b0 + plen <= 192;
  uint64_t sl0 = 0, sl1 = 0, sl2 = 0;
  if (needs_path) {
    if (win) {
      uint32_t w[12];
#pragma unroll
      for (int j = 0; j < 6; j++) {
        const uint32_t r = min(r0 + j, kPlanBmRows - 1);
        w[j] = b32[4 * kRowVec * r + C_SL];
        w[6 + j] = b32[4 * kRowVec * r + C_QM];
      }
      sl0 = w[0] | ((uint64_t)w[1] << 32);
      sl1 = w[2] | ((uint64_t)w[3] << 32);
      sl2 = w[4] | ((uint64_t)w[5] << 32);
      n = plen;
      if ((f & OSE_URL_PATH_MASK) == OSE_URL_PATH_TARGET) {
        const uint64_t q0 = (w[6] | ((uint64_t)w[7] << 32)) & half_mask(b0, b0 + plen, 0);
        const uint64_t q1 = (w[8] | ((uint64_t)w[9] << 32)) & half_mask(b0, b0 + plen, 64);
        const uint64_t q2 = (w[10] | ((uint64_t)w[11] << 32)) & half_mask(b0, b0 + plen, 128);
        if (q0) n = (uint32_t)__builtin_ctzll(q0) - b0;
        else if (q1) n = 64 + (uint32_t)__builtin_ctzll(q1) - b0;
        else if (q2) n = 128 + (uint32_t)__builtin_ctzll(q2) - b0;
      }
      p.lead = (n > 0 && ((sl0 >> b0) & 1)) ? 1 : 0;
    } else {
      n = (f & OSE_URL_PATH_MASK) == OSE_URL_PATH_TARGET ? first_of(bm, C_QM, p0, p0 + plen) - p0 : plen;
      p.lead = (n > 0 && rd.at(0) == '/') ? 1 : 0;
    }
    if (n == p.lead) {
      p.mode = M_SLASH;
      p.len = 1;
    } else {
      if (win) {
        sl0 &= half_mask(b0 + p.lead, b0 + n, 0);
        sl1 &= half_mask(b0 + p.lead, b0 + n, 64);
        sl2 &= half_mask(b0 + p.lead, b0 + n, 128);
        nseg = 1 + __builtin_popcountll(sl0) + __builtin_popcountll(sl1) + __builtin_popcountll(sl2);
      } else {
        nseg = 1 + count_of(bm, C_SL, p0 + p.lead, p0 + n);
      }
      if (cfg.n_rules && nseg <= cfg.max_rule_nseg) {
        const uint32_t* by_len = reinterpret_cast<const uint32_t*>(cfg.blob + cfg.h->rules_by_len_off);
        const UrlRuleDev* rules = reinterpret_cast<const UrlRuleDev*>(cfg.blob + cfg.h->rules_off);
        for (uint32_t r = by_len[nseg]; r < by_len[nseg + 1]; r++) {
          const int64_t l = attempt_rule(cfg, rules[r], rd, p.lead, n);
          if (l >= 0) {
            p.mode = M_RULE;
            p.field = r;
            p.len = p.lead + (uint32_t)l;
            nseg = 0;
            break;
          }
        }
      }
    }
  }
  const uint32_t incl = wave_incl_sum_u32(nseg);
  const uint32_t total = lane_value(incl, kWave - 1);
  if (total > kSegCap) return false;
  const uint32_t off = incl - nseg;
  if (nseg) {
    const uint32_t bend = p0 + n;
    uint32_t s = p0 + p.lead, k = 0;
    const uint32_t own = (uint32_t)lane << 25;
    if (win) {
      const uint32_t wb = p0 - b0;
      for (uint64_t m = sl0; m; m &= m - 1) {
        const uint32_t e = wb + (uint32_t)__builtin_ctzll(m);
        segs[off + k++] = s | ((e - s) << 12) | own;
        s = e + 1;
      }
      for (uint64_t m = sl1; m; m &= m - 1) {
        const uint32_t e = wb + 64 + (uint32_t)__builtin_ctzll(m);
        segs[off + k++] = s | ((e - s) << 12) | own;
        s = e + 1;
      }
      for (uint64_t m = sl2; m; m &= m - 1) {
        const uint32_t e = wb + 128 + (uint32_t)__builtin_ctzll(m);
        segs[off + k++] = s | ((e - s) << 12) | own;
        s = e + 1;
      }
      segs[off + k] = s | ((bend - s) << 12) | own;
    } else {
      for (; k < nseg; k++) {
        const uint32_t e = k + 1 < nseg ? first_of(bm, C_SL, s, bend) : bend;
        segs[off + k] = s | ((e - s) << 12) | own;
        s = e + 1;
      }
    }
  }
  wave_lds_sync();
  if (tm) { const uint64_t c1 = clk(); tt[0] += c1 - c0; c0 = c1; }
  LdsReader rd0(stage32, 0);
  bool longseg = false;
  auto put_cls = [&](uint32_t x, int id, uint32_t L) {
    const uint32_t nl = cfg.n_custom == 0 ? (id <= 0 ? 2u : id == 1 ? 4u : 5u)
                        : cfg.names_tab_all ? (uint32_t)cfg.name_tab[id >= 0 ? id : 0].len
                                            : (id >= 0 ? name_len(cfg, (uint32_t)id) : 0u);
    const uint32_t out = id >= 0 ? nl + 2 : L;
    cls[x] = (out << 8) | min((uint32_t)(id + 1), 255u);
  };
  for (uint32_t x0 = 0; x0 < total; x0 += kWave) {
    const uint32_t x = x0 + (uint32_t)lane;
    if (x < total) {
      const uint32_t ent = segs[x];
      const uint32_t s = ent & 0xFFFu, L = (ent >> 12) & 0x1FFFu;
      int id = -1;
      if (L <= 64)
        id = classify_spec(cfg, rd0, bm, s, s, L);
      else
        longseg = true;
      put_cls(x, id, L);
    }
  }
  wave_lds_sync();
  if (__ballot(longseg)) return false;
  if (tm) { const uint64_t c1 = clk(); tt[1] += c1 - c0; c0 = c1; }
  bool big = false;
  if (nseg) {
    uint32_t l = p.lead + nseg - 1;
    bool templated = false;
    if (nseg <= 8) {
      uint32_t r[8];
#pragma unroll
      for (uint32_t k = 0; k < 8; k++) r[k] = cls[off + k];
      uint32_t any = 0, bigm = 0, code = 0;
#pragma unroll
      for (uint32_t k = 0; k < 8; k++) {
        const uint32_t v = k < nseg ? r[k] : 0u;
        const uint32_t id1 = v & 0xFFu;
        l += v >> 8;
        any |= id1;
        bigm |= id1 > 15 ? 1u : 0u;
        code |= (id1 <= 15 ? id1 : 0u) << (4 * k);
      }
      templated = any != 0;
      big = bigm != 0;
      p.slow = big;
      p.code = code;
    } else {
      for (uint32_t k = 0; k < nseg; k++) {
        const uint32_t r = cls[off + k];
        const int id = (int)(r & 0xFFu) - 1;
        l += r >> 8;
        if (id >= 0) {
          templated = true;
          if (k < 16 && id < 15) p.code |= (uint64_t)(id + 1) << (k * 4);
          else p.slow = true;
          big |= id >= 15;
        }
      }
    }
    if (templated) { p.mode = M_DEFAULT; p.len = l; }
    else { p.mode = M_ORIG; p.len = 1 + (n - p.lead); }
    p.field = n < kNField ? n : kNField;
  }
  if (tm) tt[2] += clk() - c0;
  if (seg_off) *seg_off = off | (nseg << 16);
  if (big_id) *big_id = big;
  return true;
}

struct PlanCols {
  uint32_t f;
  ose_strref pr;
  uint32_t kind;
  bool ok;
};
__device__ __forceinline__ PlanCols plan_cols(const UrlKernelArgs& a, uint64_t i) {
  PlanCols c{0, {0, 0}, 0, false};
  if (i < a.n_spans) {
    c.f = a.url_flags[i];
    c.kind = a.kind[i];
    c.pr = a.path[i];
    c.ok = a.res_url_ok == nullptr || a.res_url_ok[a.resource[i]];
  }
  return c;
}
__device__ __forceinline__ uint32_t plan_gate(const PlanCols& c) {
  if (!c.ok || !(c.f & OSE_URL_HAS_METHOD) || (c.kind != OSE_KIND_SERVER && c.kind != OSE_KIND_CLIENT)) return 0;
  const uint32_t tgt = c.f & OSE_URL_TGT_MASK;
  if (tgt != OSE_URL_TGT_ABSENT)
    return (tgt == OSE_URL_TGT_STR_EMPTY && (c.f & OSE_URL_NAME_EQ_METHOD)) ? 1u : 0u;
  return (c.f & OSE_URL_PATH_MASK) != OSE_URL_PATH_NONE ? 2u : 0u;
}

__device__ __forceinline__ void assemble_group(lds_out_u8* img, const lds_u8* L, uint32_t stage_src, uint32_t* segs,
                                               uint32_t* cls, const BracedNames& bn, uint32_t bn_src,
                                               const Plan& p, uint32_t seg_off, uint32_t local, bool builtin) {
  const int lane = threadIdx.x & 63;
  const uint32_t nseg = seg_off >> 16, off = seg_off & 0xFFFFu;
  const uint32_t pre = (p.lead || p.mode == M_ORIG) ? 1u : 0u;
  uint32_t unused;
  const uint32_t E0 = wave_excl_scan(nseg ? p.len + 1 - pre : 0u, &unused);
  const int32_t adj = (int32_t)local - (int32_t)E0 - (int32_t)(1 - pre);
  const uint32_t pk = ((uint32_t)adj & 0xFFFFu) | (off << 16) | (pre << 24);
  if (p.len && (p.mode == M_SLASH || p.mode == M_RENAME_SLASH)) {
    img[local] = '/';
  }
  const uint32_t total = lane_value(off + nseg, kWave - 1);
  uint32_t carry = 0;
  for (uint32_t x0 = 0; x0 < total; x0 += kWave) {
    const uint32_t x = x0 + (uint32_t)lane;
    const bool v = x < total;
    const uint32_t ent = v ? segs[x] : 0u, c = v ? cls[x] : 0u;
    const uint32_t opk = (uint32_t)__shfl((int)pk, (int)(ent >> 25), kWave);
    uint32_t stot;
    const uint32_t E = carry + wave_excl_scan(v ? (c >> 8) + 1 : 0u, &stot);
    carry += stot;
    if (v) {
      const uint32_t pos = (uint32_t)(((int32_t)(opk << 16) >> 16) + (int32_t)E);
      const bool slash = x != ((opk >> 16) & 0xFFu) || (opk >> 24);
      const int id = (int)(c & 0xFFu) - 1;
      const uint32_t idc = id >= 0 ? (uint32_t)id : 0u;
      const uint32_t boff = builtin ? (idc == 0 ? 1u : idc == 1 ? 6u : 13u) : (uint32_t)bn.off[idc];
      const uint32_t blen = builtin ? (idc == 0 ? 4u : idc == 1 ? 6u : 7u) : (uint32_t)bn.len[idc];
      const uint32_t so = id >= 0 ? bn_src + boff : stage_src + (ent & 0xFFFu);
      const uint32_t n = id >= 0 ? blen : (ent >> 12) & 0x1FFFu;
      if (slash) img[pos] = '/';
      lds_out_u8* dp = img + pos + 1;
      const lds_u8* sp = L + so;
      const uint32_t nf = n & ~7u, rem = n & 7u;
#if OSE_ASM_BATCH
      const uint64_t u0 = *reinterpret_cast<const lds_u64u*>(sp), u1 = *reinterpret_cast<const lds_u64u*>(sp + 8);
      const uint64_t ut = *reinterpret_cast<const lds_u64u*>(sp + nf);
      if (nf > 0) *reinterpret_cast<lds_w64u*>(dp) = u0;
      if (nf > 8) *reinterpret_cast<lds_w64u*>(dp + 8) = u1;
      for (uint32_t q = 16; q < nf; q += 8)
        *reinterpret_cast<lds_w64u*>(dp + q) = *reinterpret_cast<const lds_u64u*>(sp + q);
      if (rem) {
        const uint64_t v = ut;
#else
      for (uint32_t q = 0; q < nf; q += 8)
        *reinterpret_cast<lds_w64u*>(dp + q) = *reinterpret_cast<const lds_u64u*>(sp + q);
      if (rem) {
        const uint64_t v = *reinterpret_cast<const lds_u64u*>(sp + nf);
#endif
        if (rem >= 4) {
          *reinterpret_cast<lds_w32u*>(dp + nf) = (uint32_t)v;
          *reinterpret_cast<lds_w32u*>(dp + n - 4) = (uint32_t)(v >> (8 * (rem - 4)));
        } else if (rem >= 2) {
          *reinterpret_cast<lds_w16u*>(dp + nf) = (uint16_t)v;
          *reinterpret_cast<lds_w16u*>(dp + n - 2) = (uint16_t)(v >> (8 * (rem - 2)));
        } else {
          dp[nf] = (uint8_t)v;
        }
      }
    }
  }
}

constexpr int kModeGeneral = 1, kModeDiag = 2;
template <int kMode>
__global__ __launch_bounds__(kThreads) __attribute__((amdgpu_waves_per_eu(4, 4))) void url_plan_kernel(UrlKernelArgs a) {
  __shared__ PlanSmem sm;
  const int lane = threadIdx.x & 63, wv = threadIdx.x >> 6;
  Cfg cfg = load_cfg(a, sm.ns);
  load_braced_names(cfg, sm.bn);
  if (!(kMode & kModeGeneral)) {
    cfg.n_custom = 0;
    cfg.n_rules = 0;
    cfg.max_rule_nseg = 0;
    cfg.names_tab_all = 1;
  }
  if (!(kMode & kModeDiag)) {
    cfg.ablate = 0;
    a.ablate = 0;
    a.dbg = nullptr;
  }
  const uint32_t stride = wave_stride();
  uint32_t g = wave_first_group();
  if (g >= a.n_groups) return;
  const bool tm = (kMode & kModeDiag) && a.dbg != nullptr;
  uint64_t t0 = 0, t_stage = 0, t_bm = 0, t_plan = 0, t_emit = 0, tt[3] = {0, 0, 0};
  const bool fused_cfg = sm.bn.ok && !(a.ablate & 2);
  const lds_u8* L = (const lds_u8*)(void*)&sm;
  const uint32_t bn_src = (uint32_t)((uint8_t*)sm.bn.b - (uint8_t*)&sm);
  uint64_t region = a.refs ? 0 : (uint64_t)wave_first_group() * a.scr_region;
  uint64_t scr_used = 0, scr_end = a.refs ? 0 : a.scr_region;
  bool exhausted = false;

  PlanCols cur = plan_cols(a, (uint64_t)g * kWave + lane);
  PlanCols nxt = plan_cols(a, (uint64_t)(g + stride) * kWave + lane);
  PlanCols nn{};
  bool np = plan_gate(cur) == 2;
  StageDma pf = stage_dma(a.arena, np ? cur.pr.off : ~0u, np ? cur.pr.off + cur.pr.len : 0u, sm.stage[wv]);
  bool first = true;
  for (;;) {
    if (tm) t0 = clk();
    wait_dma();
    if (!first) {
      cur = nxt;
      nxt = nn;
    }
    first = false;
    uint8_t* stage = sm.stage[wv];
    lds_u32* stage32 = (lds_u32*)stage;
    const uint64_t i = (uint64_t)g * kWave + lane;
    const uint32_t g2 = g + stride;
    const bool more = g2 < a.n_groups;
    const bool np2 = more && plan_gate(nxt) == 2;
    nn = plan_cols(a, (uint64_t)(g2 + stride) * kWave + lane);
    if (tm) { const uint64_t t1 = clk(); t_stage += t1 - t0; t0 = t1; }

    const uint32_t gate = plan_gate(cur);
    const bool needs_path = gate == 2;
    const uint32_t lo16 = pf.base;
    const bool staged = __ballot(lo16 == ~0u) == 0;
    if (staged && pf.bytes && !(a.ablate & 4)) {
      uint32_t m0 = 0, m1 = 0, m2 = 0;
      if (needs_path && cur.pr.len) {
        const uint32_t rl = (cur.pr.off - lo16) >> 5, rh = (cur.pr.off - lo16 + cur.pr.len - 1) >> 5;
        m0 = row_bits(rl, rh, 0);
        m1 = row_bits(rl, rh, 32);
        m2 = row_bits(rl, rh, 64);
      }
      m0 = wave_or_u32(m0);
      m1 = wave_or_u32(m1);
      m2 = wave_or_u32(m2);
      build_bitmaps_rows(stage32, (lds_u4*)sm.bm[wv], m0, m1, m2, sm.segs[wv]);
      wave_lds_sync();
    }
    if (tm) { const uint64_t t1 = clk(); t_bm += t1 - t0; t0 = t1; }
    Plan p;
    uint32_t oflags = 0;
    bool listed = false, big = false;
    uint32_t seg_off = 0;
    if (staged && !(a.ablate & (1024 | 2)))
      listed = plan_group_list(cfg, stage32, (lds_cu4*)sm.bm[wv], sm.segs[wv], needs_path, cur.pr.off - lo16,
                               cur.pr.len, cur.f, p, tm, tt, sm.cls[wv], &seg_off, &big);
    if (gate == 1) {
      p.mode = M_RENAME_SLASH;
      p.len = 1;
      oflags = OSE_OUT_RENAME;
    } else if (needs_path && (a.ablate & 2)) {
      p.mode = M_ORIG;
      p.len = 1 + cur.pr.len;
      p.field = cur.pr.len;
      oflags = OSE_OUT_SET_ATTR;
    }
    const bool unplanned = __ballot(needs_path && !listed && !(a.ablate & 2)) != 0;
    if (needs_path && !(a.ablate & 2)) {
      oflags = OSE_OUT_SET_ATTR;
      if ((cur.f & OSE_URL_NAME_EQ_METHOD) && p.len > 0) oflags |= OSE_OUT_RENAME;
    }
    if (unplanned) {
      if (lane == 0) a.unplanned[atomicAdd(a.unplanned_count, 1u)] = g;
    } else {
    uint32_t sum32;
    const uint32_t local = wave_excl_scan(p.len, &sum32);
    const uint64_t sum = sum32;
    const uint64_t need = (sum + 15) & ~15ull;
    bool fast = fused_cfg && listed && __ballot(p.mode == M_RULE || big) == 0 && sum <= kImgCap;
    if (fast && scr_used + need > scr_end) {
      if (a.refs && !exhausted) {
        const uint64_t csz = max(a.refs_chunk, need);
        uint64_t at = 0;
        if (lane == 0) at = atomicAdd((unsigned long long*)a.bump, (unsigned long long)csz);
        at = (uint64_t)lane_value((uint32_t)at, 0) | ((uint64_t)lane_value((uint32_t)(at >> 32), 0) << 32);
        const uint64_t avail = at < a.out_cap ? min(csz, a.out_cap - at) : 0;
        if (avail >= need) {
          region = at;
          scr_used = 0;
          scr_end = avail;
        } else {
          if (lane == 0) atomicCAS((unsigned long long*)a.bump, (unsigned long long)(at + csz), (unsigned long long)at);
          fast = false;
          exhausted = true;
        }
      } else {
        fast = false;
      }
    }
    if (i < a.n_spans) {
      a.plan_len[i] = p.len;
      a.url_out[i] = (uint8_t)oflags;
      if (!fast) {
        a.plan_meta[i] = pack_meta(p.mode, p.lead, p.slow, oflags, p.field);
        a.plan_code[i] = p.code;
      }
    }
    if (tm) { const uint64_t t1 = clk(); t_plan += t1 - t0; t0 = t1; }
    if (fast) {
      lds_u4* img4 = (lds_u4*)sm.bm[wv];
      const uint32_t n16 = (uint32_t)(need / 16);
      if (!(a.ablate & 64))
        assemble_group((lds_out_u8*)sm.bm[wv], L, (uint32_t)(stage - (uint8_t*)&sm), sm.segs[wv], sm.cls[wv], sm.bn,
                       bn_src, p, seg_off, local, cfg.n_custom == 0);
      wave_lds_sync();
      uint4* dst = reinterpret_cast<uint4*>(a.scratch + region + scr_used);
      for (uint32_t k = lane; k < n16; k += kWave) {
        const u32x4 v = img4[k];
        dst[k] = make_uint4(v.x, v.y, v.z, v.w);
      }
      if (lane == 0) {
        a.group_sum[g] = sum;
        a.group_scr[g] = region + scr_used;
      }
      if (a.refs && i < a.n_spans) a.tmpl[i] = ose_strref{(uint32_t)(region + scr_used + local), p.len};
      scr_used += need;
    } else {
      if (a.refs && sum == 0 && i < a.n_spans) a.tmpl[i] = ose_strref{0, 0};
      if (lane == 0) {
        a.group_sum[g] = sum;
        a.group_scr[g] = ~0ull;
        if (sum) a.slow_groups[atomicAdd(a.slow_count, 1u)] = g;
      }
    }
    }
    if (tm) { const uint64_t t1 = clk(); t_emit += t1 - t0; t0 = t1; }
    if (!more) break;
    wave_lds_sync();
    pf = stage_dma(a.arena, np2 ? nxt.pr.off : ~0u, np2 ? nxt.pr.off + nxt.pr.len : 0u, sm.stage[wv]);
    g = g2;
  }
  if (tm && lane == 0) {
    atomicAdd((unsigned long long*)&a.dbg[0], (unsigned long long)t_stage);
    atomicAdd((unsigned long long*)&a.dbg[1], (unsigned long long)t_bm);
    atomicAdd((unsigned long long*)&a.dbg[2], (unsigned long long)t_plan);
    atomicAdd((unsigned long long*)&a.dbg[3], 1ull);
    atomicAdd((unsigned long long*)&a.dbg[5], (unsigned long long)t_emit);
    atomicAdd((unsigned long long*)&a.dbg[13], (unsigned long long)tt[0]);
    atomicAdd((unsigned long long*)&a.dbg[14], (unsigned long long)tt[1]);
    atomicAdd((unsigned long long*)&a.dbg[15], (unsigned long long)tt[2]);
  }
}

constexpr int kScanThreads = 1024;
__global__ __launch_bounds__(kScanThreads) void url_scan_kernel(UrlKernelArgs a) {
  __shared__ uint64_t wsum[kScanThreads / kWave], wsum_a[kScanThreads / kWave];
  __shared__ uint64_t prefix;
  __shared__ uint32_t tile_s;
  const int tid = threadIdx.x, lane = tid & 63, wv = tid >> 6;
  if (tid == 0) tile_s = atomicAdd(a.scan_counter, 1u);
  __syncthreads();
  const uint32_t tile = tile_s;
  const uint64_t k = (uint64_t)tile * kScanThreads + tid;
  const uint64_t v = k < a.n_groups && !(a.refs && a.group_scr[k] != ~0ull) ? a.group_sum[k] : 0;
  const uint64_t sb = a.refs ? min(*a.bump, a.out_cap) : 0;
  uint64_t incl = v;
#pragma unroll
  for (int o = 1; o < kWave; o <<= 1) {
    const uint64_t t = __shfl_up(incl, o, kWave);
    if (lane >= o) incl += t;
  }
  if (lane == kWave - 1) wsum[wv] = incl;
  const uint64_t va = a.refs ? wave_sum_u64((v + 15) & ~15ull) : 0;
  if (a.refs && lane == 0) wsum_a[wv] = va;
  __syncthreads();
  uint64_t wbase = 0, total = 0;
#pragma unroll
  for (int w = 0; w < kScanThreads / kWave; w++) {
    const uint64_t x = wsum[w];
    if (w < wv) wbase += x;
    total += x;
  }
  if (wv == 0) {
    if (a.refs && lane == 0) {
      uint64_t ta = 0;
      for (int w = 0; w < kScanThreads / kWave; w++) ta += wsum_a[w];
      if (ta) atomicAdd((unsigned long long*)a.slow_aligned, (unsigned long long)ta);
    }
    const uint64_t pfx = lookback_prefix(a.scan_status, tile, total, a.error);
    if (lane == 0) {
      prefix = pfx;
      if (tile == a.n_scan_tiles - 1) {
        const bool over = sb + pfx + total > a.out_cap;
        uint64_t used = sb + pfx + total;
        if (over && a.refs) {
          const uint64_t X = sb + __hip_atomic_load((unsigned long long*)a.slow_aligned, __ATOMIC_RELAXED,
                                                    __HIP_MEMORY_SCOPE_AGENT);
          used = 2 * X + (uint64_t)kImgCap * min(a.plan_waves, kUrlMaxWaves);
        }
        if (a.used) *a.used = used;
        if (over) atomicOr(a.error, 2u);
      }
    }
  }
  __syncthreads();
  if (k < a.n_groups) a.group_base[k] = sb + prefix + wbase + incl - v;
}

struct CopyCols {
  uint32_t len;
  uint64_t base, gsum, so;
};
__device__ __forceinline__ CopyCols copy_cols(const UrlKernelArgs& a, uint32_t g, int lane) {
  CopyCols c{0, 0, 0, ~0ull};
  const uint64_t i = (uint64_t)g * kWave + lane;
  c.base = a.group_base[g];
  c.gsum = a.group_sum[g];
  c.so = a.group_scr[g];
  if (i < a.n_spans) c.len = a.plan_len[i];
  return c;
}
__device__ __forceinline__ CopyCols copy_len(const UrlKernelArgs& a, uint32_t g, int lane) {
  CopyCols c{0, 0, 0, ~0ull};
  const uint64_t i = (uint64_t)g * kWave + lane;
  if (i < a.n_spans) c.len = a.plan_len[i];
  return c;
}
__device__ __forceinline__ void copy_round(uint8_t* gdst, uint32_t shift, uint64_t endb, uint32_t c0, uint32_t nchunk,
                                           const uint4& v, uint32_t& carry) {
  const int lane = threadIdx.x & 63;
  const uint32_t c = c0 + (uint32_t)lane;
  uint32_t pw = (uint32_t)__shfl_up((int)v.w, 1, kWave);
  if (lane == 0) pw = carry;
  carry = lane_value(v.w, kWave - 1);
  const uint32_t sh = 4 - shift;
  const uint32_t w0 = shift ? __builtin_amdgcn_alignbyte(v.x, pw, sh) : v.x;
  const uint32_t w1 = shift ? __builtin_amdgcn_alignbyte(v.y, v.x, sh) : v.y;
  const uint32_t w2 = shift ? __builtin_amdgcn_alignbyte(v.z, v.y, sh) : v.z;
  const uint32_t w3 = shift ? __builtin_amdgcn_alignbyte(v.w, v.z, sh) : v.w;
  if (c < nchunk) {
    const uint64_t b0 = 16ull * c;
    if (b0 >= shift && b0 + 16 <= endb) {
      uint32_t* d = reinterpret_cast<uint32_t*>(gdst + b0);
      d[0] = w0;
      d[1] = w1;
      d[2] = w2;
      d[3] = w3;
    } else {
      const uint32_t ws[4] = {w0, w1, w2, w3};
#pragma unroll
      for (uint32_t q = 0; q < 16; q++)
        if (b0 + q >= shift && b0 + q < endb) gdst[b0 + q] = (uint8_t)(ws[q >> 2] >> (8 * (q & 3)));
    }
  }
}
struct CopyJob {
  const uint4* src;
  uint8_t* gdst;
  uint32_t shift, n16, nchunk;
  uint64_t endb;
  bool on;
};
__device__ __forceinline__ CopyJob copy_job(const UrlKernelArgs& a, const CopyCols& c) {
  CopyJob j{};
  j.on = c.so != ~0ull && c.gsum != 0 && c.base + c.gsum <= a.out_cap;
  if (!j.on) return j;
  j.src = reinterpret_cast<const uint4*>(a.scratch + c.so);
  j.shift = (uint32_t)(c.base & 3);
  j.gdst = a.out_arena + (c.base - j.shift);
  j.endb = j.shift + c.gsum;
  j.n16 = (uint32_t)((c.gsum + 15) / 16);
  j.nchunk = (uint32_t)((j.endb + 15) / 16);
  return j;
}
__device__ __forceinline__ uint4 copy_load(const CopyJob& j, uint32_t c0) {
  const uint32_t c = c0 + (threadIdx.x & 63);
  return j.on && c < j.n16 ? j.src[c] : make_uint4(0, 0, 0, 0);
}
__device__ __forceinline__ void copy_rest(const CopyJob& j, uint4 v, uint32_t& carry) {
  copy_round(j.gdst, j.shift, j.endb, 0, j.nchunk, v, carry);
  for (uint32_t c0 = kWave; c0 < j.nchunk; c0 += kWave) {
    v = copy_load(j, c0);
    copy_round(j.gdst, j.shift, j.endb, c0, j.nchunk, v, carry);
  }
}
template <bool kSize, bool kRefs>
__global__ __launch_bounds__(kThreads) __attribute__((amdgpu_waves_per_eu(kSize ? 5 : 6, 8))) void url_copy_kernel(UrlKernelArgs a) {
  static_assert(kSize || !kRefs, "the refs form has no copy pass");
  const int lane = threadIdx.x & 63;
  const uint32_t stride = wave_stride();
  uint32_t kept = 0;
  const bool sz_on = kSize && !sizedev::size_batch_dropped(a.sz);
  uint32_t g = wave_first_group();
  if (kRefs && !sz_on) g = a.n_groups;
  CopyCols An{0, 0, 0, ~0ull};
  sizedev::SpanCols xn{};
  if (g < a.n_groups) {
    An = kRefs ? copy_len(a, g, lane) : copy_cols(a, g, lane);
    if (kSize && sz_on) xn = sizedev::size_span_load(a.sz, (uint64_t)g * kWave + lane, false);
  }
  for (; g < a.n_groups; g += stride) {
    const uint64_t ia = (uint64_t)g * kWave + lane;
    const CopyCols A = An;
    const sizedev::SpanCols x0 = xn;
    const bool more = g + stride < a.n_groups;
    if (more) {
      An = kRefs ? copy_len(a, g + stride, lane) : copy_cols(a, g + stride, lane);
      if (kSize && sz_on) xn = sizedev::size_span_load(a.sz, (uint64_t)(g + stride) * kWave + lane, false);
    }
    sizedev::SpanCols x = x0;
    CopyJob ja{};
    uint4 va = make_uint4(0, 0, 0, 0);
    if (!kRefs) {
      uint32_t unused;
      const uint32_t la = wave_excl_scan(A.len, &unused);
      ja = copy_job(a, A);
      va = copy_load(ja, 0);
      if (ia < a.n_spans) a.tmpl[ia] = ose_strref{(uint32_t)(A.base + la), A.len};
    }
    if (kSize && sz_on) {
      x.tl = A.len;
      kept += sizedev::size_span_finish(a.sz, x);
    }
    uint32_t carry = 0;
    if (!kRefs && ja.on) copy_rest(ja, va, carry);
    if (!more) break;
  }
  if (kSize) {
    __shared__ uint32_t wk[kWaves];
#pragma unroll
    for (int o = 32; o > 0; o >>= 1) kept += __shfl_xor(kept, o, kWave);
    if (lane == 0) wk[threadIdx.x >> 6] = kept;
    __syncthreads();
    if (threadIdx.x == 0) {
      uint32_t t = 0;
      for (int w = 0; w < kWaves; w++) t += wk[w];
      a.size_partials[blockIdx.x] = t;
    }
  }
}
struct SlowPlanSmem {
  NamesSmem ns;
  __attribute__((aligned(16))) uint8_t stage[kPlanStage + 16];
  __attribute__((aligned(16))) u32x4 bm[kRowVec * kPlanBmRows];
  uint32_t segs[kSegCap];
  uint32_t cls[kSegCap + 8];
};
__global__ __launch_bounds__(kWave) void url_plan_slow_kernel(UrlKernelArgs a) {
  __shared__ SlowPlanSmem sm;
  const uint32_t count = *a.unplanned_count;
  if (blockIdx.x >= count) return;
  const int lane = threadIdx.x;
  const uint64_t c0 = a.dbg ? clk() : 0;
  const Cfg cfg = load_cfg(a, sm.ns);
  uint64_t c_plan = 0;
  const uint64_t c1 = a.dbg ? clk() : 0;
  lds_u32* stage32 = (lds_u32*)sm.stage;
  uint64_t tt[3] = {0, 0, 0};
  for (uint32_t k = blockIdx.x; k < count; k += gridDim.x) {
    const uint32_t g = a.unplanned[k];
    const uint64_t i = (uint64_t)g * kWave + lane;
    const PlanCols c = plan_cols(a, i);
    const uint32_t gate = plan_gate(c);
    Plan p;
    uint32_t oflags = 0;
    if (gate == 1) {
      p.mode = M_RENAME_SLASH;
      p.len = 1;
      oflags = OSE_OUT_RENAME;
    }
    const uint32_t lo_l = c.pr.off, hi_l = c.pr.off + c.pr.len;
    const uint32_t nc = gate == 2 && c.pr.len ? ((hi_l + 15u) >> 4) - (lo_l >> 4) : 0u;
    bool todo = gate == 2;
    while (__ballot(todo)) {
      const uint64_t t = a.dbg ? clk() : 0;
      uint32_t unused;
      const uint32_t cs = wave_excl_scan(todo ? nc : 0u, &unused);
      bool take = todo && cs + nc <= kPlanStage / 16;
      const bool alone = __ballot(take) == 0;
      if (alone) {
        const int first = __builtin_ctzll(__ballot(todo));
        if (lane == first) {
          p = plan_global(cfg, a.arena + c.pr.off, c.pr.len, c.f);
          todo = false;
        }
        continue;
      }
      const StageDma sd = stage_dma(a.arena, take ? lo_l : ~0u, take ? hi_l : 0u, sm.stage);
      wait_dma();
      const uint32_t p0 = c.pr.off - sd.base;
      uint32_t m0 = 0, m1 = 0, m2 = 0;
      if (take && c.pr.len) {
        const uint32_t rl = p0 >> 5, rh = (p0 + c.pr.len - 1) >> 5;
        m0 = row_bits(rl, rh, 0);
        m1 = row_bits(rl, rh, 32);
        m2 = row_bits(rl, rh, 64);
      }
      build_bitmaps_rows(stage32, (lds_u4*)sm.bm, wave_or_u32(m0), wave_or_u32(m1), wave_or_u32(m2), sm.segs);
      wave_lds_sync();
      Plan q;
      const bool listed = plan_group_list(cfg, stage32, (lds_cu4*)sm.bm, sm.segs, take, p0, c.pr.len, c.f, q, false,
                                          tt, sm.cls);
      if (take) {
        if (listed) {
          p = q;
        } else {
          LdsReader rd(stage32, p0);
          p = plan_path(cfg, rd, c.pr.len, c.f);
        }
        todo = false;
      }
      wave_lds_sync();
      if (a.dbg) c_plan += clk() - t;
    }
    if (gate == 2) {
      oflags = OSE_OUT_SET_ATTR;
      if ((c.f & OSE_URL_NAME_EQ_METHOD) && p.len > 0) oflags |= OSE_OUT_RENAME;
    }
    if (i < a.n_spans) {
      a.plan_len[i] = p.len;
      a.url_out[i] = (uint8_t)oflags;
      a.plan_meta[i] = pack_meta(p.mode, p.lead, p.slow, oflags, p.field);
      a.plan_code[i] = p.code;
    }
    const uint64_t sum = wave_sum_u64(p.len);
    if (a.refs && sum == 0 && i < a.n_spans) a.tmpl[i] = ose_strref{0, 0};
    if (lane == 0) {
      a.group_sum[g] = sum;
      a.group_scr[g] = ~0ull;
      if (sum) a.slow_groups[atomicAdd(a.slow_count, 1u)] = g;
    }
  }
  if (a.dbg) {
    const uint64_t c2 = clk();
    if (lane == 0) {
      atomicMax((unsigned long long*)&a.dbg[8], (unsigned long long)(c1 - c0));
      atomicMax((unsigned long long*)&a.dbg[9], (unsigned long long)(c2 - c0));
      atomicMax((unsigned long long*)&a.dbg[10], (unsigned long long)c_plan);
    }
  }
}

struct EmitSlowSmem {
  NamesSmem ns;
  __attribute__((aligned(16))) uint8_t stage[kWaves][kStage + 16];
  __attribute__((aligned(16))) uint32_t img[kWaves][kWaveOut / 4 + 4];
};
__global__ __launch_bounds__(kThreads) void url_emit_slow_kernel(UrlKernelArgs a) {
  __shared__ EmitSlowSmem sm;
  const uint32_t count = *a.slow_count;
  if (blockIdx.x * kWaves >= count) return;
  const int lane = threadIdx.x & 63, wv = threadIdx.x >> 6;
  const Cfg cfg = load_cfg(a, sm.ns);
  uint8_t* stage = sm.stage[wv];
  lds_u32* stage32 = (lds_u32*)stage;
  lds_w32* img = (lds_w32*)sm.img[wv];
  for (uint32_t k = wave_first_group(); k < count; k += wave_stride()) {
    const uint32_t g = a.slow_groups[k];
    const uint64_t i = (uint64_t)g * kWave + lane;
    const EmitCols c = emit_cols(a, g, lane);
    const uint64_t base = c.base, gtotal = c.gsum;
    const uint32_t len = c.len, meta = c.meta, mode = meta & 7u;
    uint32_t unused;
    const uint32_t local = wave_excl_scan(len, &unused);
    if (a.refs && i < a.n_spans) a.tmpl[i] = ose_strref{(uint32_t)(base + local), len};
    if (base + gtotal > a.out_cap) continue;
    const bool needs_path = emit_needs_path(meta);
    const ose_strref pr = needs_path ? c.pr : ose_strref{0, 0};
    uint32_t nbytes;
    const uint32_t lo16 = stage_wave(stage, a.arena, needs_path ? pr.off : ~0u, needs_path ? pr.off + pr.len : 0u,
                                     &nbytes);
    const uint32_t shift = (uint32_t)(base & 3);
    const uint32_t img_bytes = shift + (uint32_t)gtotal;
    const bool direct = img_bytes > kWaveOut || lo16 == ~0u;
    if (!direct) {
      for (uint32_t k2 = lane; k2 < (img_bytes + 3) / 4; k2 += kWave) img[k2] = 0;
      wave_lds_sync();
    }
    if (len) {
      const uint32_t lead = (meta >> 3) & 1u, field = meta >> 7;
      const bool slow = (meta >> 4) & 1u;
      const uint32_t f = (needs_path && (mode == M_RULE || field == kNField)) ? a.url_flags[i] : 0u;
      if (!direct) {
        PutOr put(img, shift + local);
        LdsReader rd(stage32, pr.off - lo16);
        emit_path(cfg, rd, pr.len, f, mode, lead, slow, field, c.code, put);
        put.finish();
      } else if (lo16 != ~0u) {
        emit_out_of_line(cfg, LdsReader(stage32, pr.off - lo16), pr.len, f, mode, lead, slow, field, c.code,
                         a.out_arena + base + local, len);
      } else {
        emit_out_of_line(cfg, ByteReader(a.arena + pr.off), pr.len, f, mode, lead, slow, field, c.code,
                         a.out_arena + base + local, len);
      }
    }
    wave_lds_sync();
    if (!direct) store_image(a, img, base, shift, gtotal);
    wave_lds_sync();
  }
}

__global__ __launch_bounds__(kThreads) void url_nfa_fill_kernel(UrlKernelArgs a) {
  const uint32_t k = blockIdx.x * kThreads + threadIdx.x;
  if (k < a.n_groups) a.unplanned[k] = k;
  if (k == 0) *a.unplanned_count = a.n_groups;
}

struct NfaPlanSmem {
  NamesSmem ns;
  __attribute__((aligned(16))) uint8_t stage[kStage + 16];
};
__global__ __launch_bounds__(kWave) void url_nfa_plan_kernel(UrlKernelArgs a) {
  __shared__ NfaPlanSmem sm;
  const uint32_t count = *a.unplanned_count;
  if (blockIdx.x >= count) return;
  const int lane = threadIdx.x;
  const Cfg cfg = load_cfg(a, sm.ns);
  lds_u32* stage32 = (lds_u32*)sm.stage;
  const NfaState nx{a.nfa_slab + (uint64_t)blockIdx.x * 2 * a.nfa_words * kWave + lane};
  for (uint32_t k = blockIdx.x; k < count; k += gridDim.x) {
    const uint32_t g = a.unplanned[k];
    const uint64_t i = (uint64_t)g * kWave + lane;
    const PlanCols c = plan_cols(a, i);
    const uint32_t gate = plan_gate(c);
    Plan p;
    uint32_t oflags = 0;
    if (gate == 1) {
      p.mode = M_RENAME_SLASH;
      p.len = 1;
      oflags = OSE_OUT_RENAME;
    }
    const bool reads = gate == 2 && c.pr.len;
    uint32_t nbytes;
    const uint32_t lo16 = stage_wave(sm.stage, a.arena, reads ? c.pr.off : ~0u, reads ? c.pr.off + c.pr.len : 0u, &nbytes);
    if (gate == 2) {
      if (lo16 != ~0u) {
        LdsReader rd(stage32, reads ? c.pr.off - lo16 : 0u);
        p = plan_path(cfg, rd, c.pr.len, c.f, nx);
      } else {
        p = plan_global_nfa(cfg, a.arena + c.pr.off, c.pr.len, c.f, nx);
      }
      oflags = OSE_OUT_SET_ATTR;
      if ((c.f & OSE_URL_NAME_EQ_METHOD) && p.len > 0) oflags |= OSE_OUT_RENAME;
    }
    wave_lds_sync();
    if (i < a.n_spans) {
      a.plan_len[i] = p.len;
      a.url_out[i] = (uint8_t)oflags;
      a.plan_meta[i] = pack_meta(p.mode, p.lead, p.slow, oflags, p.field);
      a.plan_code[i] = p.code;
    }
    const uint64_t sum = wave_sum_u64(p.len);
    if (a.refs && sum == 0 && i < a.n_spans) a.tmpl[i] = ose_strref{0, 0};
    if (lane == 0) {
      a.group_sum[g] = sum;
      a.group_scr[g] = ~0ull;
      if (sum) a.slow_groups[atomicAdd(a.slow_count, 1u)] = g;
    }
  }
}

__global__ __launch_bounds__(kThreads) void url_nfa_emit_kernel(UrlKernelArgs a) {
  __shared__ EmitSlowSmem sm;
  const uint32_t count = *a.slow_count;
  if (blockIdx.x * kWaves >= count) return;
  const int lane = threadIdx.x & 63, wv = threadIdx.x >> 6;
  const Cfg cfg = load_cfg(a, sm.ns);
  uint8_t* stage = sm.stage[wv];
  lds_u32* stage32 = (lds_u32*)stage;
  lds_w32* img = (lds_w32*)sm.img[wv];
  const NfaState nx{a.nfa_slab + (uint64_t)(blockIdx.x * kWaves + wv) * 2 * a.nfa_words * kWave + lane};
  for (uint32_t k = wave_first_group(); k < count; k += wave_stride()) {
    const uint32_t g = a.slow_groups[k];
    const uint64_t i = (uint64_t)g * kWave + lane;
    const EmitCols c = emit_cols(a, g, lane);
    const uint64_t base = c.base, gtotal = c.gsum;
    const uint32_t len = c.len, meta = c.meta, mode = meta & 7u;
    uint32_t unused;
    const uint32_t local = wave_excl_scan(len, &unused);
    if (a.refs && i < a.n_spans) a.tmpl[i] = ose_strref{(uint32_t)(base + local), len};
    if (base + gtotal > a.out_cap) continue;
    const bool needs_path = emit_needs_path(meta);
    const ose_strref pr = needs_path ? c.pr : ose_strref{0, 0};
    uint32_t nbytes;
    const uint32_t lo16 = stage_wave(stage, a.arena, needs_path ? pr.off : ~0u, needs_path ? pr.off + pr.len : 0u,
                                     &nbytes);
    const uint32_t shift = (uint32_t)(base & 3);
    const uint32_t img_bytes = shift + (uint32_t)gtotal;
    const bool direct = img_bytes > kWaveOut || lo16 == ~0u;
    if (!direct) {
      for (uint32_t k2 = lane; k2 < (img_bytes + 3) / 4; k2 += kWave) img[k2] = 0;
      wave_lds_sync();
    }
    if (len) {
      const uint32_t lead = (meta >> 3) & 1u, field = meta >> 7;
      const bool slow = (meta >> 4) & 1u;
      const uint32_t f = (needs_path && (mode == M_RULE || field == kNField)) ? a.url_flags[i] : 0u;
      if (!direct) {
        PutOr put(img, shift + local);
        LdsReader rd(stage32, pr.off - lo16);
        emit_path(cfg, rd, pr.len, f, mode, lead, slow, field, c.code, put, nx);
        put.finish();
      } else if (lo16 != ~0u) {
        emit_out_of_line(cfg, LdsReader(stage32, pr.off - lo16), pr.len, f, mode, lead, slow, field, c.code,
                         a.out_arena + base + local, len, nx);
      } else {
        emit_out_of_line(cfg, ByteReader(a.arena + pr.off), pr.len, f, mode, lead, slow, field, c.code,
                         a.out_arena + base + local, len, nx);
      }
    }
    wave_lds_sync();
    if (!direct) store_image(a, img, base, shift, gtotal);
    wave_lds_sync();
  }
}

template <class K>
static uint32_t resident_blocks(K kernel, size_t dyn_lds) {
  int dev = 0, cus = 0, per_cu = 0;
  if (hipGetDevice(&dev) != hipSuccess) return 1024;
  if (hipDeviceGetAttribute(&cus, hipDeviceAttributeMultiprocessorCount, dev) != hipSuccess || cus <= 0) cus = 256;
  if (hipOccupancyMaxActiveBlocksPerMultiprocessor(&per_cu, kernel, kThreads, dyn_lds) != hipSuccess || per_cu <= 0)
    per_cu = 2;
  return (uint32_t)(cus * per_cu);
}

}

static int url_mode(const UrlKernelArgs& a) {
  return (a.general ? kModeGeneral : 0) | ((OSE_DIAG && (a.ablate || a.dbg)) ? kModeDiag : 0);
}
template <int M>
static uint32_t plan_blocks(const UrlKernelArgs& a) {
  static const uint32_t res = resident_blocks(url_plan_kernel<M>, 0);
  const uint32_t cap = a.refs && a.plan_grid_mult > 1 ? res * a.plan_grid_mult : std::min<uint32_t>(res, kUrlMaxWaves / kWaves);
  return std::min<uint32_t>(cap, (a.n_groups + kWaves - 1) / kWaves);
}
template <int M>
static void launch_plan_mode(const UrlKernelArgs& a, hipStream_t st) {
  hipLaunchKernelGGL(url_plan_kernel<M>, dim3(plan_blocks<M>(a)), dim3(kThreads), 0, st, a);
}
uint64_t url_refs_chunk(uint64_t cap, uint32_t waves) {
  return std::min<uint64_t>(256 << 10, cap / 8 / std::max<uint32_t>(1, waves)) & ~15ull;
}
uint32_t url_plan_waves(const UrlKernelArgs& a) {
  switch (url_mode(a)) {
    case 0: return plan_blocks<0>(a) * kWaves;
#if OSE_DIAG
    case 2: return plan_blocks<2>(a) * kWaves;
    case 3: return plan_blocks<3>(a) * kWaves;
#endif
    default: return plan_blocks<1>(a) * kWaves;
  }
}
void launch_url_plan(const UrlKernelArgs& a, hipStream_t st) {
  switch (url_mode(a)) {
    case 0: launch_plan_mode<0>(a, st); break;
#if OSE_DIAG
    case 2: launch_plan_mode<2>(a, st); break;
    case 3: launch_plan_mode<3>(a, st); break;
#endif
    default: launch_plan_mode<1>(a, st); break;
  }
}
void launch_url_scan(const UrlKernelArgs& a, hipStream_t st) {
  hipLaunchKernelGGL(url_scan_kernel, dim3(a.n_scan_tiles), dim3(kScanThreads), 0, st, a);
}
uint32_t url_copy_blocks(uint32_t n_groups) {
  return std::max<uint32_t>(1, std::min<uint32_t>(kUrlCopyMaxBlocks, (n_groups + 2 * kWaves - 1) / (2 * kWaves)));
}
void launch_url_copy(const UrlKernelArgs& a, hipStream_t st) {
  const uint32_t blocks = url_copy_blocks(a.n_groups);
  if (a.refs) {
    if (a.fuse_size) hipLaunchKernelGGL((url_copy_kernel<true, true>), dim3(blocks), dim3(kThreads), 0, st, a);
  } else if (a.fuse_size) {
    hipLaunchKernelGGL((url_copy_kernel<true, false>), dim3(blocks), dim3(kThreads), 0, st, a);
  } else {
    hipLaunchKernelGGL((url_copy_kernel<false, false>), dim3(blocks), dim3(kThreads), 0, st, a);
  }
}
void launch_url_plan_slow(const UrlKernelArgs& a, hipStream_t st) {
  static const uint32_t cap = [] {
    int dev = 0, cus = 0, per_cu = 0;
    if (hipGetDevice(&dev) != hipSuccess) return 1024u;
    if (hipDeviceGetAttribute(&cus, hipDeviceAttributeMultiprocessorCount, dev) != hipSuccess || cus <= 0) cus = 256;
    if (hipOccupancyMaxActiveBlocksPerMultiprocessor(&per_cu, url_plan_slow_kernel, kWave, 0) != hipSuccess || per_cu <= 0)
      per_cu = 2;
    return (uint32_t)(cus * per_cu);
  }();
  const uint32_t blocks = std::min<uint32_t>(cap, a.n_groups);
  if (blocks) hipLaunchKernelGGL(url_plan_slow_kernel, dim3(blocks), dim3(kWave), 0, st, a);
}
void launch_url_emit_slow(const UrlKernelArgs& a, hipStream_t st) {
  static const uint32_t cap = resident_blocks(url_emit_slow_kernel, 0);
  const uint32_t blocks = std::min<uint32_t>(cap, (a.n_groups + kWaves - 1) / kWaves);
  hipLaunchKernelGGL(url_emit_slow_kernel, dim3(blocks), dim3(kThreads), 0, st, a);
}

void launch_url_nfa_fill(const UrlKernelArgs& a, hipStream_t st) {
  hipLaunchKernelGGL(url_nfa_fill_kernel, dim3((a.n_groups + kThreads - 1) / kThreads), dim3(kThreads), 0, st, a);
}
void launch_url_nfa_plan(const UrlKernelArgs& a, hipStream_t st) {
  static const uint32_t cap = [] {
    int dev = 0, cus = 0, per_cu = 0;
    if (hipGetDevice(&dev) != hipSuccess) return 1024u;
    if (hipDeviceGetAttribute(&cus, hipDeviceAttributeMultiprocessorCount, dev) != hipSuccess || cus <= 0) cus = 256;
    if (hipOccupancyMaxActiveBlocksPerMultiprocessor(&per_cu, url_nfa_plan_kernel, kWave, 0) != hipSuccess || per_cu <= 0)
      per_cu = 2;
    return (uint32_t)(cus * per_cu);
  }();
  const uint32_t blocks = std::min<uint32_t>({cap, a.n_groups, url_nfa_waves(a.n_spans)});
  if (blocks) hipLaunchKernelGGL(url_nfa_plan_kernel, dim3(blocks), dim3(kWave), 0, st, a);
}
void launch_url_nfa_emit(const UrlKernelArgs& a, hipStream_t st) {
  static const uint32_t cap = resident_blocks(url_nfa_emit_kernel, 0);
  const uint32_t blocks =
      std::min<uint32_t>({cap, (a.n_groups + kWaves - 1) / kWaves, url_nfa_waves(a.n_spans) / kWaves});
  hipLaunchKernelGGL(url_nfa_emit_kernel, dim3(blocks), dim3(kThreads), 0, st, a);
}

}
```

odigos_amd/native.py:

```python
from __future__ import annotations

import ctypes as C
import os
from pathlib import Path

LIB_PATH = Path(__file__).resolve().parent / "_lib" / "libodigos_amd.so"

OSE_OK = 0
OSE_EINVAL = -22
OSE_ENOMEM = -12
OSE_ENOTSUP = -95
OSE_EDEVICE = -5
OSE_ERANGE = -34
OSE_ETIMEDOUT = -110
OSE_NONE = 0xFFFFFFFF

KIND_UNSPECIFIED, KIND_INTERNAL, KIND_SERVER, KIND_CLIENT, KIND_PRODUCER, KIND_CONSUMER = range(6)
STATUS_UNSET, STATUS_OK, STATUS_ERROR = range(3)

URL_HAS_METHOD = 0x01
URL_TGT_MASK = 0x06
URL_TGT_ABSENT = 0x00
URL_TGT_STR_EMPTY = 0x02
URL_TGT_STR = 0x04
URL_TGT_NONSTR = 0x06
URL_NAME_EQ_METHOD = 0x08
URL_PATH_MASK = 0x30
URL_PATH_NONE = 0x00
URL_PATH_RAW = 0x10
URL_PATH_TARGET = 0x20

DB_HAS_QUERY = 0x01
DB_HAS_OPNAME = 0x02
SQLOP_NONE, SQLOP_SELECT, SQLOP_INSERT, SQLOP_UPDATE, SQLOP_DELETE, SQLOP_CREATE, SQLOP_DROP, SQLOP_ALTER = range(8)
SQLOP_NAMES = ("UNKNOWN", "SELECT", "INSERT", "UPDATE", "DELETE", "CREATE", "DROP", "ALTER")

OUT_SET_ATTR = 0x01
OUT_RENAME = 0x02

STAGE_SAMPLE = 0x1
STAGE_TEMPLATE = 0x2
STAGE_SIZE = 0x4
STAGE_APPLY_KEEP = 0x8
STAGE_TEMPLATE_REFS = 0x10
STAGE_APPLY_TEMPLATE = 0x20
STAGE_SQLOP = 0x40
STAGE_APPLY_SQLOP = 0x80
STAGE_CONDATTR = 0x100
CA_KEEP, CA_ARENA, CA_CONFIG = range(3)
XREC_BYTES = 56

GROUP_TRACE_ID = 0
GROUP_BATCH = 1

ATTR_ABSENT, ATTR_STR, ATTR_INT, ATTR_DOUBLE, ATTR_BOOL, ATTR_OTHER = range(6)

_p = C.c_void_p


class StrRef(C.Structure):
    _fields_ = [("off", C.c_uint32), ("len", C.c_uint32)]


class Rand(C.Structure):
    _fields_ = [("seed", C.c_uint64), ("traffic_u", C.c_double)]


COLUMN_FIELDS = [
    "arena", "trace_id", "start_ns", "end_ns", "status", "kind", "resource", "scope", "url_flags",
    "path", "route", "span_size", "name_len", "route_match", "attr_match", "res_svc", "res_svc_str", "res_url_ok", "res_attrset",
    "res_size", "scope_size", "scope_resource",
]


class Columns(C.Structure):
    _fields_ = [
        ("n_spans", C.c_uint64), ("n_resources", C.c_uint32), ("n_scopes", C.c_uint32),
        ("n_attrsets", C.c_uint32), ("attr_match_words", C.c_uint32), ("arena_bytes", C.c_uint64),
    ] + [(f, _p) for f in COLUMN_FIELDS] + [("svc_match", _p), ("n_attr_keys", C.c_uint32), ("match_planes", C.c_uint32),
                                            ("attr_type", _p), ("attr_val", _p),
                                            ("db_flags", _p), ("db_query", _p), ("res_sql_ok", _p)]


class Outputs(C.Structure):
    _fields_ = [
        ("keep", _p), ("trace_count", _p), ("trace_first_span", _p), ("trace_keep", _p),
        ("trace_level", _p), ("trace_ratio", _p),
        ("url_out", _p), ("tmpl", _p), ("tmpl_arena", _p), ("tmpl_arena_cap", C.c_uint64),
        ("tmpl_arena_used", _p),
        ("attrset_bytes", _p), ("accepted_spans", _p), ("res_bytes", _p),
        ("device_status", _p),
        ("sql_op", _p),
    ]


class CondAttrInfo(C.Structure):
    _fields_ = [("n_rules", C.c_uint32), ("n_keys", C.c_uint32), ("n_targets", C.c_uint32), ("string_bytes", C.c_uint32)]


class CondAttrColumns(C.Structure):
    _fields_ = [("n_spans", C.c_uint64), ("n_resources", C.c_uint32), ("n_scopes", C.c_uint32), ("arena_bytes", C.c_uint64)] + [
        (f, _p) for f in ("arena", "scope", "scope_resource", "scope_name", "span_has", "span_val", "span_kv_size",
                          "scope_has", "scope_val", "res_has", "res_val", "span_size")]


class CondAttrOutputs(C.Structure):
    _fields_ = [(f, _p) for f in ("src", "val", "span_size_out", "scratch", "device_status")]


class EngineInfo(C.Structure):
    _fields_ = [("stages", C.c_uint32), ("max_template_name", C.c_uint32),
                ("inverse_sampling", C.c_int64), ("traffic_sampling_ratio", C.c_double),
                ("n_attr_rules", C.c_uint32), ("n_attr_keys", C.c_uint32), ("attr_host_rules", C.c_uint64)]


_lib = None


def lib() -> C.CDLL:
    global _lib
    if _lib is not None:
        return _lib
    path = LIB_PATH
    variant = os.environ.get("OSE_LIB_VARIANT", "")
    if variant:
        path = LIB_PATH.with_name(f"libodigos_amd{variant}.so")
    if not path.exists():
        raise RuntimeError(f"{path} is missing: run `python -m odigos_amd.build` (hipcc, gfx950)")
    try:
        import torch
    except ImportError:
        pass
    L = C.CDLL(str(path))
    sig = {
        "ose_last_error": (C.c_char_p, []),
        "ose_engine_create": (C.c_int, [C.c_char_p, C.POINTER(_p)]),
        "ose_engine_destroy": (None, [_p]),
        "ose_dropped_errors": (C.c_uint64, [C.c_char_p, C.c_size_t]),
        "ose_engine_service_id": (C.c_uint32, [_p, C.c_char_p, C.c_size_t]),
        "ose_engine_get_info": (C.c_int, [_p, C.POINTER(EngineInfo)]),
        "ose_set_device": (C.c_int, [C.c_int]),
        "ose_otlp_decode": (C.c_int, [_p, _p, C.c_size_t, _p, C.POINTER(_p)]),
        "ose_host_alloc": (C.c_int, [C.c_size_t, C.POINTER(_p)]),
        "ose_host_free": (None, [_p]),
        "ose_otlp_columns": (C.POINTER(Columns), [_p]),
        "ose_otlp_host_spans": (C.c_uint32, [_p]),
        "ose_otlp_walk_info": (C.c_int, [_p, C.POINTER(C.c_uint32)]),
        "ose_otlp_timings": (C.c_int, [_p, C.POINTER(C.c_double)]),
        "ose_otlp_attrset": (C.c_int, [_p, C.c_uint32, C.c_char_p, C.c_size_t]),
        "ose_otlp_download": (C.c_int, [_p, C.POINTER(Columns)]),
        "ose_otlp_release": (None, [_p]),
        "ose_router_create": (C.c_int, [C.c_char_p, C.POINTER(_p)]),
        "ose_router_destroy": (None, [_p]),
        "ose_router_pipelines": (C.c_uint32, [_p]),
        "ose_router_pipeline": (C.c_char_p, [_p, C.c_uint32]),
        "ose_otlp_encode": (C.c_int, [_p, _p, C.POINTER(Outputs), C.c_uint32, C.c_uint32, _p, _p, C.POINTER(_p)]),
        "ose_otlp_out_count": (C.c_uint32, [_p]),
        "ose_otlp_out_get": (C.c_int, [_p, C.c_uint32, C.POINTER(C.c_char_p), C.POINTER(_p),
                                       C.POINTER(C.c_uint64), C.POINTER(C.c_uint32)]),
        "ose_otlp_out_release": (None, [_p]),
        "ose_gbt_create": (C.c_int, [_p, C.c_char_p, C.c_uint64, C.c_uint64, C.POINTER(_p)]),
        "ose_gbt_destroy": (None, [_p]),
        "ose_gbt_add": (C.c_int, [_p, C.POINTER(Columns), _p, C.c_int64, _p]),
        "ose_gbt_release": (C.c_int, [_p, C.c_int64, _p, C.POINTER(C.POINTER(Columns)), C.POINTER(C.c_uint32)]),
        "ose_gbt_stats": (C.c_int, [_p, C.POINTER(C.c_uint64)]),
        "ose_gbt_download": (C.c_int, [_p, C.POINTER(Columns)]),
        "ose_gbt_add_otlp": (C.c_int, [_p, _p, _p, C.c_int64, _p]),
        "ose_gbt_release_otlp": (C.c_int, [_p, C.c_int64, _p, C.POINTER(_p), C.POINTER(C.c_uint32)]),
        "ose_engine_attr_key": (C.c_int, [_p, C.c_uint32, C.POINTER(C.c_char_p), C.POINTER(C.c_uint32)]),
        "ose_engine_attr_host_rules": (C.c_uint32, [_p, C.POINTER(C.c_uint64), C.c_uint32]),
        "ose_otlp_pipeline_create": (C.c_int, [_p, _p, C.c_uint32, C.c_uint64, C.POINTER(_p)]),
        "ose_otlp_pipeline_consume": (C.c_int, [_p, C.c_void_p, C.c_size_t, C.c_void_p, C.POINTER(_p)]),
        "ose_otlp_pipeline_counters": (C.c_int, [_p, C.c_char_p, C.c_size_t]),
        "ose_otlp_pipeline_destroy": (None, [_p]),
        "osehost_otlp_pipeline_hold": (C.c_int, [_p, C.c_uint32]),
        "osehost_otlp_pipeline_tune": (C.c_int, [_p, C.c_uint32, C.c_uint32, C.c_uint32]),
        "ose_engine_path_counts": (C.c_uint32, [_p, C.POINTER(C.c_uint64), C.c_uint32]),
        "ose_engine_url_nfa_groups": (C.c_uint64, [_p]),
        "ose_engine_set_option": (C.c_int, [_p, C.c_char_p, C.c_int64]),
        "ose_batch_acquire": (C.c_int, [_p, C.POINTER(Columns), C.POINTER(_p)]),
        "ose_batch_columns": (C.POINTER(Columns), [_p]),
        "ose_batch_outputs": (C.POINTER(Outputs), [_p]),
        "ose_batch_release": (None, [_p]),
        "ose_process": (C.c_int, [_p, _p, C.c_uint32, C.c_uint32, C.POINTER(Rand)]),
        "ose_process_device": (C.c_int, [_p, C.POINTER(Columns), C.POINTER(Outputs), C.c_uint32, C.c_uint32,
                                         C.POINTER(Rand), _p]),
        "ose_reserve": (C.c_int, [_p, C.c_uint64, C.c_uint64]),
        "ose_device_info": (C.c_int, [C.c_char_p, C.c_size_t]),
        "ose_shard_owner": (C.c_uint32, [C.c_uint64, C.c_uint64, C.c_uint32]),
        "ose_shard_pack": (C.c_int, [_p, C.POINTER(Columns), C.c_uint32, _p, _p, _p, _p]),
        "ose_shard_unpack": (C.c_int, [_p, C.c_uint64, C.c_uint32, _p, _p, _p, _p, _p, _p, _p, _p, _p, _p]),
        "ose_shard_decide": (C.c_int, [_p, _p, C.c_uint64, C.c_uint32, _p, _p, _p, _p]),
        "ose_shard_record_bytes": (C.c_uint32, [_p]),
        "ose_shard_scatter_keep": (C.c_int, [_p, _p, C.c_uint64, _p, _p]),
        "ose_nccl_unique_id": (C.c_int, [_p, C.c_size_t]),
        "ose_nccl_comm_init": (C.c_int, [C.POINTER(_p), C.c_int, _p, C.c_int]),
        "ose_nccl_comm_destroy": (None, [_p]),
        "ose_exchange_sample": (C.c_int, [_p, C.POINTER(Columns), C.POINTER(Outputs), _p, C.c_int, C.c_int,
                                          C.POINTER(Rand), _p, _p]),
        "ose_allreduce_counters": (C.c_int, [_p, _p, C.c_uint64, _p, _p]),
        "ose_engine_condattr_info": (C.c_int, [_p, C.POINTER(CondAttrInfo)]),
        "ose_engine_condattr_key": (C.c_int, [_p, C.c_uint32, C.POINTER(_p), C.POINTER(C.c_uint32), C.POINTER(C.c_uint32)]),
        "ose_engine_condattr_string": (C.c_int, [_p, C.POINTER(_p), C.POINTER(C.c_uint32)]),
        "ose_condattr_scratch_words": (C.c_uint64, [_p, C.c_uint32]),
        "ose_condattr_process_device": (C.c_int, [_p, C.POINTER(CondAttrColumns), C.POINTER(CondAttrOutputs), _p]),
        "ose_condattr_process": (C.c_int, [_p, C.POINTER(CondAttrColumns), C.POINTER(CondAttrOutputs)]),
        "ose_otlp_condattr_columns": (C.POINTER(CondAttrColumns), [_p]),
        "ose_otlp_condattr_download": (C.c_int, [_p, C.POINTER(CondAttrColumns)]),
        "ose_otlp_encode_condattr": (C.c_int, [_p, _p, C.POINTER(CondAttrOutputs), _p, _p, C.POINTER(_p)]),
        "ose_profile_enable": (C.c_int, [_p, C.c_int]),
        "ose_profile_read": (C.c_int, [_p, C.c_char_p, C.c_size_t]),
        "osehost_last_error": (C.c_char_p, []),
        "osehost_sampling_chunks": (C.c_int, [C.c_char_p, C.POINTER(C.c_uint32)]),
        "osehost_sampling_layout": (C.c_uint32, [C.c_uint64, C.POINTER(C.c_uint64), C.POINTER(C.c_uint64), C.c_uint32,
                                                 C.POINTER(C.c_uint64)]),
        "osehost_url_layout": (C.c_uint32, [C.c_uint64, C.c_uint64, C.c_uint32, C.c_int, C.POINTER(C.c_uint64),
                                            C.POINTER(C.c_uint64), C.c_uint32, C.POINTER(C.c_uint64),
                                            C.POINTER(C.c_uint64)]),
        "osehost_stage_offsets": (None, [C.c_uint32, C.c_int, C.c_uint64, C.c_uint64, C.c_uint64, C.c_uint64, C.c_uint32,
                                         C.POINTER(C.c_uint64)]),
        "osehost_gbt_copy_times": (C.c_int, [_p, C.c_int, C.POINTER(C.c_double)]),
        "osehost_gbt_state": (C.c_int, [_p, C.POINTER(C.c_uint64), C.c_uint32]),
        "osehost_gbt_layout": (C.c_uint32, [C.c_uint32, C.c_uint64, C.c_uint64, C.c_uint64, C.c_uint64, C.c_uint32, C.c_int,
                                            C.POINTER(C.c_uint64), C.POINTER(C.c_uint64), C.c_uint32,
                                            C.POINTER(C.c_uint64)]),
        "osehost_stream_copy": (C.c_int, [_p, _p, C.c_size_t, C.c_int, _p, C.POINTER(C.c_double)]),
        "osehost_xgroup_create": (C.c_int, [C.c_int, C.POINTER(_p)]),
        "osehost_owner_last_general": (C.c_uint32, [_p]),
        "osehost_xgroup_destroy": (None, [_p]),
        "osehost_exchange_sample_local": (C.c_int, [_p, C.POINTER(Columns), C.POINTER(Outputs), _p, C.c_int,
                                                    C.POINTER(Rand), _p, C.POINTER(C.c_uint64)]),
        "osehost_allreduce_counters_local": (C.c_int, [_p, _p, C.c_uint64, _p, C.c_int, _p]),
        "osehost_processor_create": (_p, [C.c_char_p, C.c_char_p]),
        "osehost_processor_destroy": (None, [_p]),
        "osehost_processor_set": (None, [_p, C.c_uint64, C.c_uint32]),
        "osehost_consume": (C.c_int, [_p, C.c_char_p, C.POINTER(_p)]),
        "osehost_columnarize": (_p, [_p, C.c_char_p]),
        "osehost_batch_columns": (C.POINTER(Columns), [_p]),
        "osehost_batch_outputs": (C.POINTER(Outputs), [_p]),
        "osehost_apply": (C.c_int, [_p, _p, C.POINTER(_p)]),
        "osehost_bench": (C.c_int, [_p, C.c_char_p, C.c_uint32, C.c_uint32, C.POINTER(C.c_double)]),
        "osehost_batch_free": (None, [_p]),
        "osehost_metrics_json": (_p, [_p]),
        "osehost_roundtrip": (_p, [C.c_char_p]),
        "osehost_pb_to_json": (_p, [C.c_char_p, C.c_size_t]),
        "osehost_otlp_walk": (_p, [C.c_char_p, C.c_char_p, C.c_size_t]),
        "osehost_otlp_encode": (C.c_int, [C.c_char_p, C.c_size_t, _p, C.c_int, _p, _p, _p, C.c_uint64, _p, C.c_int,
                                          C.POINTER(_p)]),
        "osehost_otlp_encode_sql": (C.c_int, [C.c_char_p, C.c_size_t, _p, C.c_int, _p, _p, _p, C.c_uint64, _p, C.c_int,
                                              C.POINTER(_p), _p]),
        "osehost_otlp_encode_condattr": (C.c_int, [C.c_char_p, C.c_size_t, C.c_uint64, _p, _p, C.c_uint32, _p, C.c_uint64,
                                                   _p, C.c_uint64, _p, _p, _p, C.c_int, C.POINTER(_p)]),
        "osehost_router_create_signal": (C.c_int, [C.c_char_p, C.c_char_p, C.POINTER(_p)]),
        "osehost_router_route": (_p, [_p, C.c_char_p]),
        "osehost_router_table": (C.c_int, [_p, _p, C.c_size_t, C.POINTER(C.c_uint64), C.POINTER(C.c_uint32),
                                           C.POINTER(C.c_uint64)]),
        "osehost_otlp_out_timings": (C.c_int, [_p, C.POINTER(C.c_double)]),
        "osehost_otlp_out_path": (C.c_int, [_p, C.POINTER(C.c_uint32)]),
        "osehost_parse_duration": (C.c_int, [C.c_char_p, C.POINTER(C.c_int64)]),
        "osehost_resource_sizes": (C.c_int, [C.c_char_p, C.c_int, C.POINTER(C.c_uint64), C.c_size_t]),
        "osehost_as_string": (_p, [C.c_char_p]),
        "osehost_free": (None, [_p]),
        "osehost_regex_match": (C.c_int, [C.c_char_p, C.c_char_p, C.c_size_t]),
        "osehost_regex_nfa_match": (C.c_int, [C.c_char_p, C.c_char_p, C.c_size_t]),
        "osehost_regex_nfa_size": (C.c_int, [C.c_char_p]),
        "osehost_url_blob_hash": (C.c_int, [C.c_char_p, C.c_int, C.POINTER(C.c_uint64), C.POINTER(C.c_uint64),
                                            C.POINTER(C.c_uint32)]),
        "osehost_regex_match_host": (C.c_int, [C.c_char_p, C.c_char_p, C.c_size_t, C.c_uint32, C.c_uint64,
                                               C.POINTER(C.c_int)]),
        "osehost_span_attr_eval": (C.c_int, [C.c_char_p, C.c_char_p]),
        "osehost_sqlop_detect": (C.c_uint32, [C.c_char_p, C.c_size_t]),
        "osehost_condattr_compile": (C.c_int, [C.c_char_p, C.POINTER(CondAttrInfo), C.POINTER(_p)]),
        "osehost_condattr_blob": (C.c_int, [C.c_char_p, C.POINTER(_p), C.POINTER(C.c_size_t)]),
        "osehost_condattr_span": (C.c_int, [C.c_char_p, C.POINTER(CondAttrColumns), C.POINTER(CondAttrOutputs)]),
        "osehost_batch_condattr_columns": (C.POINTER(CondAttrColumns), [_p]),
        "osehost_batch_condattr_outputs": (C.POINTER(CondAttrOutputs), [_p]),
    }
    for name, (res, args) in sig.items():
        fn = getattr(L, name)
        fn.restype = res
        fn.argtypes = args
    _lib = L
    return L


def exported_symbols() -> list[str]:
    import re
    hdr = (Path(__file__).resolve().parent.parent / "include" / "odigos_amd.h").read_text()
    return sorted(set(re.findall(r"^\s*(?:[\w\s\*]+?)\b(ose_\w+)\s*\(", hdr, re.M)))


def last_error() -> str:
    return (lib().ose_last_error() or b"").decode("utf-8", "replace")


def take_bytes(ptr) -> bytes:
    if not ptr:
        raise RuntimeError((lib().osehost_last_error() or b"").decode("utf-8", "replace"))
    b = C.string_at(ptr)
    lib().osehost_free(ptr)
    return b


class OseError(RuntimeError):
    def __init__(self, code: int, msg: str):
        super().__init__(f"ose error {code}: {msg}")
        self.code = code


def check(rc: int) -> None:
    if rc != 0:
        raise OseError(rc, last_error())
```

Baseline: 14.65 billion spans/s.

## Slice URL plan and fused copy into staggered chunks across two streams

Splits the URL-template plan and fused copy/size tail into group-range slices. Plans run alternately on a second stream, and each slice's copy waits only on its own slice event, so copying early slices overlaps planning of later ones. Kernels now take g_begin/g_end ranges, per-slice unplanned counters summed atomically, and per-slice size partial offsets. This adds extra launches, events and a workspace memset, and may reduce per-kernel occupancy.

```diff
diff --git a/odigos_amd/csrc/engine.cpp b/odigos_amd/csrc/engine.cpp
--- a/odigos_amd/csrc/engine.cpp
+++ b/odigos_amd/csrc/engine.cpp
@@ -62,7 +62,9 @@
   for (void* f : fold)
     if (f) (void)hipFree(f);
   if (dup_host) (void)hipHostFree(dup_host);
-  for (hipEvent_t ev : {pending, dup_ready, fork, join, join2})
+  for (hipEvent_t ev : {pending, dup_ready, fork, join, join2, fork2})
+    if (ev) (void)hipEventDestroy(ev);
+  for (hipEvent_t ev : slice_ev)
     if (ev) (void)hipEventDestroy(ev);
 }
 
@@ -293,18 +295,33 @@
     const hipError_t jw = je == hipSuccess ? hipStreamWaitEvent(st, ev, 0) : je;
     if (jw != hipSuccess) {
       (void)hipStreamSynchronize(ust);
+      if (ust2) (void)hipStreamSynchronize(ust2);
       if (!rc) rc = fail(OSE_EDEVICE, std::string("URL stream join: ") + hipGetErrorString(jw));
     }
+  }
+  hipStream_t ust2 = nullptr;
+  uint32_t open_slices(uint32_t k, uint32_t form) {
+    static_assert(sizeof(ws->slice_ev) / sizeof(ws->slice_ev[0]) == kUrlMaxSlices, "an event per slice");
+    if (k > kUrlMaxSlices) k = kUrlMaxSlices;
+    for (uint32_t s = 0; s < k; s++)
+      if (!ws->slice_ev[s] && hipEventCreateWithFlags(&ws->slice_ev[s], hipEventDisableTiming) != hipSuccess) return 1;
+    if (form == kUrlStaggered && k > 1) {
+      if (!ws->fork2) (void)hipEventCreateWithFlags(&ws->fork2, hipEventDisableTiming);
+      if (ws->fork2) ust2 = e->take_stream();
+    }
+    return k;
   }
   void close() {
     if (ust) e->give_stream(ust);
-    ust = nullptr;
+    if (ust2) e->give_stream(ust2);
+    ust = ust2 = nullptr;
   }
 };
 
-void fuse_size_into_copy(UrlKernelArgs& ua, SizeKernelArgs& sa, Workspace* ws, size_t size_off, const ose_columns* c) {
+void fuse_size_into_copy(UrlKernelArgs& ua, SizeKernelArgs& sa, Workspace* ws, size_t size_off, const ose_columns* c,
+                         const UrlSlices* S = nullptr) {
   sa.kept_partials = size_partials_of(ws, size_off, c->n_scopes, c->n_resources);
-  sa.n_kept_partials = url_copy_blocks(ua.n_groups);
+  sa.n_kept_partials = S ? S->part[S->k] : url_copy_blocks(ua.n_groups);
   ua.fuse_size = 1;
   ua.size_partials = const_cast<uint32_t*>(sa.kept_partials);
   ua.sz = sa;
@@ -359,17 +376,30 @@
   UrlFork fork{e, ws, st};
   static const bool one_stream = getenv("OSE_ONE_STREAM") != nullptr;
   constexpr uint64_t kForkSpans = 1u << 20;
-  if (!one_stream && !rc && defer && n >= kForkSpans) fork.open();
+  const bool refs_fused = tmpl && (mask & OSE_STAGE_TEMPLATE_REFS) && (mask & OSE_STAGE_SIZE) && fused_size_ok;
+  const uint32_t forced_k = e->url_tail_slices_opt.load(std::memory_order_relaxed);
+  const uint32_t plan_groups = (uint32_t)((n + kUrlGroup - 1) / kUrlGroup);
+  const uint32_t want_slices = refs_fused && !e->url_words() ? (forced_k ? forced_k : url_tail_slices(plan_groups)) : 1u;
+  const bool forks = !one_stream && !rc && defer && (n >= kForkSpans || (forced_k && refs_fused && !e->url_words()));
+  if (forks && want_slices > 1) rc = clear_url_slice_words(e, c, ws, so.url_off, st);
+  if (forks && !rc) fork.open();
   ws->beside_url = fork.ust && tmpl;
 #ifndef OSE_URL_JOIN_LATE
-  fork.early_join = fork.ust && tmpl && (mask & OSE_STAGE_TEMPLATE_REFS) && (mask & OSE_STAGE_SIZE) && fused_size_ok;
+  fork.early_join = fork.ust && refs_fused;
 #endif
-  const uint32_t plan_groups = (uint32_t)((n + kUrlGroup - 1) / kUrlGroup);
   UrlRun ur;
   ur.ws_off = so.url_off;
   ur.refs = (mask & OSE_STAGE_TEMPLATE_REFS) != 0;
   ur.grid_mult = url_plan_grid_mult(plan_groups, fork.ust != nullptr);
   ur.planned = fork.early_join ? ws->join : nullptr;
+  const uint32_t form_opt = e->url_tail_form_opt.load(std::memory_order_relaxed);
+  const uint32_t form = form_opt ? form_opt - 1 : kUrlTailForm;
+  const uint32_t slices = fork.early_join && want_slices > 1 ? fork.open_slices(want_slices, form) : 1u;
+  ur.slices = slices;
+  ur.form = form;
+  ur.slice_ev = ws->slice_ev;
+  ur.st2 = fork.ust2;
+  ur.fork2 = ws->fork2;
   if (fork.ust && tmpl) {
     rc = run_url(e, c, o, fork.ust, ws, ur, &ua);
     fork.join_recorded = fork.early_join && !rc;
@@ -384,12 +414,22 @@
     const int trc = sample_tail();
     if (!rc) rc = trc;
   }
-  if (fork.ust) fork.join(ws->join, fork.join_recorded, rc);
+  const bool sliced = slices > 1 && fork.join_recorded;
+  if (fork.ust2 && !sliced) (void)hipStreamSynchronize(fork.ust2);
+  if (fork.ust && !sliced) fork.join(ws->join, fork.join_recorded, rc);
   if (!rc && (mask & OSE_STAGE_SQLOP)) rc = run_sqlop(e, c, o, st);
   SizeKernelArgs sa{};
   bool size_on = false;
   if (!rc && (mask & OSE_STAGE_SIZE)) rc = prepare_size(e, c, o, mask, group_mode, rnd, st, ws, so.size_off, sa, size_on);
-  if (!rc && tmpl) {
+  if (sliced) {
+    const UrlSlices S = url_slices(ua.n_groups, slices, form);
+    if (!rc && size_on && n > 0) fuse_size_into_copy(ua, sa, ws, so.size_off, c, &S);
+    for (uint32_t s = 0; s < S.k; s++) {
+      if (S.g[s] == S.g[s + 1]) continue;
+      fork.join(ws->slice_ev[s], true, rc);
+      if (!rc) rc = run_url_back_slice(e, ua, S, s, st);
+    }
+  } else if (!rc && tmpl) {
     if (size_on && n > 0 && fused_size_ok) fuse_size_into_copy(ua, sa, ws, so.size_off, c);
     rc = run_url_back(e, ua, st);
   }
@@ -609,6 +649,16 @@
       {"otlp_condattr", Engine::kOptOtlpCondattr},
       {"url_regex_nfa", Engine::kOptUrlRegexNfa},
   };
+  if (strcmp(name, "url_tail_slices") == 0) {
+    if (value < 0 || value > (int64_t)kUrlMaxSlices) return fail(OSE_EINVAL, "engine option url_tail_slices: 0 to 8");
+    e->url_tail_slices_opt.store((uint32_t)value);
+    return 0;
+  }
+  if (strcmp(name, "url_tail_form") == 0) {
+    if (value < 0 || value > 2) return fail(OSE_EINVAL, "engine option url_tail_form: 0 (the rule), 1 in order, 2 staggered");
+    e->url_tail_form_opt.store((uint32_t)value);
+    return 0;
+  }
   for (const auto& o : kOpts) {
     if (strcmp(name, o.name) != 0) continue;
     if (o.bit == Engine::kOptOtlpSqlop && !e->has_sqlop)
diff --git a/odigos_amd/csrc/engine_internal.hpp b/odigos_amd/csrc/engine_internal.hpp
--- a/odigos_amd/csrc/engine_internal.hpp
+++ b/odigos_amd/csrc/engine_internal.hpp
@@ -109,6 +109,8 @@
   uint32_t* dup_host = nullptr;
   hipEvent_t dup_ready = nullptr;
   hipEvent_t fork = nullptr, join = nullptr, join2 = nullptr;
+  hipEvent_t slice_ev[8] = {};
+  hipEvent_t fork2 = nullptr;
   bool beside_url = false;
   Workspace() = default;
   Workspace(const Workspace&) = delete;
@@ -143,6 +145,7 @@
   };
   std::atomic<uint32_t> options{0};
   bool option(uint32_t o) const { return (options.load(std::memory_order_relaxed) & o) != 0; }
+  std::atomic<uint32_t> url_tail_slices_opt{0}, url_tail_form_opt{0};
   bool url_needs_resource = false;
   int64_t inverse = 1;
   uint32_t max_name = 5;
@@ -260,6 +263,7 @@
 int prepare_size(Engine* e, const ose_columns* c, const ose_outputs* o, uint32_t mask, uint32_t group_mode,
                  const ose_rand* rnd, hipStream_t st, Workspace* ws, size_t off, SizeKernelArgs& a, bool& active);
 uint32_t* size_partials_of(Workspace* ws, size_t off, uint64_t n_scopes, uint64_t n_resources);
+uint32_t size_partials_cap();
 int run_size_tail(Engine* e, const SizeKernelArgs& a, hipStream_t st);
 int run_size_scopes(Engine* e, const SizeKernelArgs& a, hipStream_t st);
 size_t size_scratch_bytes(uint64_t n_scopes, uint64_t n_resources);
@@ -290,9 +294,18 @@
   bool refs = false;
   uint32_t grid_mult = 1;
   hipEvent_t planned = nullptr;
-};
+  uint32_t slices = 1;
+  uint32_t form = 0;
+  hipEvent_t* slice_ev = nullptr;
+  hipStream_t st2 = nullptr;
+  hipEvent_t fork2 = nullptr;
+};
+struct UrlSlices;
 int run_url(Engine* e, const ose_columns* c, const ose_outputs* o, hipStream_t st, Workspace* ws, const UrlRun& r,
             UrlKernelArgs* front);
 int run_url_back(Engine* e, const UrlKernelArgs& a, hipStream_t st);
+int clear_url_slice_words(Engine* e, const ose_columns* c, Workspace* ws, size_t ws_off, hipStream_t st);
+UrlKernelArgs url_slice_args(const UrlKernelArgs& a, const UrlSlices& S, uint32_t s);
+int run_url_back_slice(Engine* e, const UrlKernelArgs& a, const UrlSlices& S, uint32_t s, hipStream_t st);
 
 }
diff --git a/odigos_amd/csrc/kernels.hpp b/odigos_amd/csrc/kernels.hpp
--- a/odigos_amd/csrc/kernels.hpp
+++ b/odigos_amd/csrc/kernels.hpp
@@ -48,7 +48,7 @@
 
 struct UrlKernelArgs {
   uint64_t n_spans;
-  uint32_t n_groups;
+  uint32_t g_begin, g_end;
   const uint8_t* arena;
   const uint8_t* url_flags;
   const uint8_t* kind;
@@ -68,6 +68,7 @@
   uint64_t* group_scr;
   uint64_t* group_sum;
   uint64_t* group_base;
+  uint32_t n_groups;
   uint32_t n_scan_tiles;
   uint32_t* scan_counter;
   uint64_t* scan_status;
@@ -91,6 +92,8 @@
   uint32_t fuse_size;
   uint32_t* size_partials;
   SizeKernelArgs sz;
+  uint32_t copy_blocks, partial_off;
+  uint32_t* unplanned_total;
 };
 constexpr uint32_t kUrlCopyMaxBlocks = 65536;
 uint32_t url_copy_blocks(uint32_t n_groups);
@@ -119,6 +122,35 @@
   const uint32_t m = n_groups / (kUrlMaxWaves * 19u);
   return m < 1 ? 1u : m > 16 ? 16u : m;
 }
+enum : uint32_t { kUrlInOrder = 0, kUrlStaggered = 1 };
+constexpr uint32_t kUrlMaxSlices = 8;
+constexpr uint32_t kUrlStaggerNum = 1, kUrlStaggerDen = 2;
+struct UrlSlices {
+  uint32_t k;
+  uint32_t g[kUrlMaxSlices + 1];
+  uint32_t part[kUrlMaxSlices + 1];
+};
+inline uint32_t url_slice_copy_blocks(uint32_t groups, uint32_t k) {
+  if (k <= 1) return url_copy_blocks(groups);
+  const uint32_t want = (groups + 7) / 8, cap = kUrlCopyMaxBlocks / k;
+  return groups == 0 ? 0u : want < cap ? want : cap;
+}
+inline UrlSlices url_slices(uint32_t n_groups, uint32_t k, uint32_t form) {
+  UrlSlices s{};
+  s.k = k < 1 ? 1u : k > kUrlMaxSlices ? kUrlMaxSlices : k;
+  const uint64_t first = form == kUrlStaggered ? kUrlStaggerNum : 1, each = form == kUrlStaggered ? kUrlStaggerDen : 1;
+  const uint64_t d = first + (s.k - 1) * each;
+  for (uint32_t j = 1; j < s.k; j++) {
+    const uint64_t num = (uint64_t)n_groups * (first + (j - 1) * each);
+    s.g[j] = (uint32_t)((num + d - 1) / d);
+  }
+  s.g[s.k] = n_groups;
+  for (uint32_t j = 0; j < s.k; j++) s.part[j + 1] = s.part[j] + url_slice_copy_blocks(s.g[j + 1] - s.g[j], s.k);
+  return s;
+}
+constexpr uint32_t kUrlTailForm = kUrlStaggered;
+constexpr uint32_t kUrlTailGroups = 1u << 20;
+inline uint32_t url_tail_slices(uint32_t n_groups) { return n_groups >= kUrlTailGroups ? 2u : 1u; }
 void launch_url_plan(const UrlKernelArgs& a, hipStream_t st);
 uint32_t url_plan_waves(const UrlKernelArgs& a);
 uint64_t url_refs_chunk(uint64_t cap, uint32_t waves);
diff --git a/odigos_amd/csrc/size_host.cpp b/odigos_amd/csrc/size_host.cpp
--- a/odigos_amd/csrc/size_host.cpp
+++ b/odigos_amd/csrc/size_host.cpp
@@ -9,6 +9,7 @@
 namespace {
 struct SizeLayout {
   size_t scope, parts, fix, partials, end;
+  uint32_t n_partials;
 };
 SizeLayout size_layout(uint64_t n_scopes) {
   const uint64_t W = (std::max<uint64_t>(n_scopes, 1) + 63) / 64;
@@ -17,7 +18,8 @@
   L.parts = up(L.scope + 8 * std::max<uint64_t>(n_scopes, 1));
   L.fix = up(L.parts + 32 * W);
   L.partials = up(L.fix + 4 * W);
-  L.end = up(L.partials + 4ull * kUrlCopyMaxBlocks) + 256;
+  L.n_partials = kUrlCopyMaxBlocks;
+  L.end = up(L.partials + 4ull * L.n_partials) + 256;
   return L;
 }
 }
@@ -91,6 +93,8 @@
   return reinterpret_cast<uint32_t*>(static_cast<uint8_t*>(ws->dev) + off + size_layout(n_scopes).partials);
 }
 
+uint32_t size_partials_cap() { return size_layout(1).n_partials; }
+
 int run_size_tail(Engine* e, const SizeKernelArgs& a, hipStream_t st) {
   if (!a.kept_partials)
     if (const int rc = e->timed("size_span_kernel", st, [&] { launch_size_spans(a, st); })) return rc;
diff --git a/odigos_amd/csrc/url_host.cpp b/odigos_amd/csrc/url_host.cpp
--- a/odigos_amd/csrc/url_host.cpp
+++ b/odigos_amd/csrc/url_host.cpp
@@ -184,6 +184,8 @@
   UrlKernelArgs a{};
   a.n_spans = n;
   a.n_groups = (uint32_t)((n + kUrlGroup - 1) / kUrlGroup);
+  a.g_begin = 0;
+  a.g_end = a.n_groups;
   a.arena = c->arena;
   a.url_flags = c->url_flags;
   a.kind = c->kind;
@@ -231,16 +233,40 @@
   return a;
 }
 
-int queue_url_front(Engine* e, const UrlKernelArgs& a, hipStream_t st, hipEvent_t planned) {
+constexpr size_t kSliceWordBytes = 64;
+static_assert(4 * (1 + kUrlMaxSlices) <= kSliceWordBytes, "a count word per slice and their sum");
+uint32_t* url_slice_words(uint8_t* base, const UrlLayout& L) { return reinterpret_cast<uint32_t*>(base + L.dbg.off + 128); }
+
+int queue_url_plan(Engine* e, const UrlKernelArgs& a, hipStream_t st) {
   int rc;
   if (a.nfa) {
     if ((rc = e->timed("url_nfa_fill_kernel", st, [&] { launch_url_nfa_fill(a, st); }))) return rc;
-    if ((rc = e->timed("url_nfa_plan_kernel", st, [&] { launch_url_nfa_plan(a, st); }))) return rc;
-  } else {
-    if ((rc = e->timed("url_plan_kernel", st, [&] { launch_url_plan(a, st); }))) return rc;
-    if ((rc = e->timed("url_plan_slow_kernel", st, [&] { launch_url_plan_slow(a, st); }))) return rc;
-  }
-  if (planned) HIP_TRY(hipEventRecord(planned, st));
+    return e->timed("url_nfa_plan_kernel", st, [&] { launch_url_nfa_plan(a, st); });
+  }
+  if ((rc = e->timed("url_plan_kernel", st, [&] { launch_url_plan(a, st); }))) return rc;
+  return e->timed("url_plan_slow_kernel", st, [&] { launch_url_plan_slow(a, st); });
+}
+
+int queue_url_slices(Engine* e, const UrlKernelArgs& a, const UrlSlices& S, const UrlRun& r, hipStream_t st) {
+  const bool two = r.form == kUrlStaggered && r.st2 && r.fork2;
+  if (two) {
+    HIP_TRY(hipEventRecord(r.fork2, st));
+    HIP_TRY(hipStreamWaitEvent(r.st2, r.fork2, 0));
+  }
+  hipEvent_t last2 = nullptr;
+  for (uint32_t s = 0; s < S.k; s++) {
+    if (S.g[s] == S.g[s + 1]) continue;
+    hipStream_t ss = two && (s & 1) ? r.st2 : st;
+    if (const int rc = queue_url_plan(e, url_slice_args(a, S, s), ss)) return rc;
+    HIP_TRY(hipEventRecord(r.slice_ev[s], ss));
+    if (ss != st) last2 = r.slice_ev[s];
+  }
+  if (last2) HIP_TRY(hipStreamWaitEvent(st, last2, 0));
+  return 0;
+}
+
+int queue_url_rest(Engine* e, const UrlKernelArgs& a, hipStream_t st) {
+  int rc;
   if ((rc = e->timed("url_scan_kernel", st, [&] { launch_url_scan(a, st); }))) return rc;
   rc = e->timed(a.nfa ? "url_nfa_emit_kernel" : "url_emit_slow_kernel", st, [&] {
     if (a.nfa) launch_url_nfa_emit(a, st);
@@ -248,7 +274,8 @@
   });
   if (rc) return rc;
   if ((e->options.load() & Engine::kOptUrlPathCounts) && e->path_count_dev) {
-    HIP_TRY(hipMemcpyAsync(e->path_count_dev + 2, a.unplanned_count, 4, hipMemcpyDeviceToDevice, st));
+    const uint32_t* unplanned = a.unplanned_total ? a.unplanned_total : a.unplanned_count;
+    HIP_TRY(hipMemcpyAsync(e->path_count_dev + 2, unplanned, 4, hipMemcpyDeviceToDevice, st));
     HIP_TRY(hipMemcpyAsync(e->path_count_dev + 3, a.slow_count, 4, hipMemcpyDeviceToDevice, st));
     if (a.nfa) HIP_TRY(hipMemcpyAsync(e->path_count_dev + 4, a.unplanned_count, 4, hipMemcpyDeviceToDevice, st));
     else HIP_TRY(hipMemsetAsync(e->path_count_dev + 4, 0, 8, st));
@@ -300,9 +327,48 @@
     a.dbg = reinterpret_cast<uint64_t*>(base + L.dbg.off);
     HIP_TRY(hipMemsetAsync(a.dbg, 0, 256, st));
   }
-  rc = queue_url_front(e, a, st, r.planned);
+  if (r.slices > 1 && r.refs && !a.nfa && r.slice_ev) {
+    const UrlSlices S = url_slices(a.n_groups, r.slices, r.form);
+    a.unplanned_total = url_slice_words(base, L);
+    uint32_t waves = 0;
+    for (uint32_t s = 0; s < S.k; s++)
+      if (S.g[s] < S.g[s + 1]) waves += url_plan_waves(url_slice_args(a, S, s));
+    a.plan_waves = waves;
+    a.refs_chunk = url_refs_chunk(o->tmpl_arena_cap, waves);
+    *front = a;
+    rc = queue_url_slices(e, a, S, r, st);
+  } else {
+    rc = queue_url_plan(e, a, st);
+    if (!rc && r.planned) HIP_TRY(hipEventRecord(r.planned, st));
+  }
+  if (!rc) rc = queue_url_rest(e, a, st);
   if (!rc) *front = a;
   return rc;
+}
+
+UrlKernelArgs url_slice_args(const UrlKernelArgs& a, const UrlSlices& S, uint32_t s) {
+  UrlKernelArgs x = a;
+  x.g_begin = S.g[s];
+  x.g_end = S.g[s + 1];
+  x.plan_grid_mult = url_plan_grid_mult(x.g_end - x.g_begin, true);
+  x.unplanned = a.unplanned + x.g_begin;
+  x.unplanned_count = a.unplanned_total + 1 + s;
+  x.copy_blocks = S.part[s + 1] - S.part[s];
+  x.partial_off = S.part[s];
+  return x;
+}
+
+int clear_url_slice_words(Engine* e, const ose_columns* c, Workspace* ws, size_t ws_off, hipStream_t st) {
+  const UrlLayout L = url_layout(c->n_spans, c->arena_bytes, e->url_words(), true);
+  if (const int rc = ws->reserve(ws_off + L.end)) return rc;
+  HIP_TRY(hipMemsetAsync(url_slice_words(static_cast<uint8_t*>(ws->dev) + ws_off, L), 0, kSliceWordBytes, st));
+  return 0;
+}
+
+int run_url_back_slice(Engine* e, const UrlKernelArgs& a, const UrlSlices& S, uint32_t s, hipStream_t st) {
+  if (S.g[s] == S.g[s + 1] || !a.fuse_size) return 0;
+  const UrlKernelArgs x = url_slice_args(a, S, s);
+  return e->timed("url_copy_kernel", st, [&] { launch_url_copy(x, st); });
 }
 
 int run_url_back(Engine* e, const UrlKernelArgs& a, hipStream_t st) {
@@ -320,6 +386,20 @@
                                        uint64_t* bytes, uint32_t cap, uint64_t* end, uint64_t* workspace_bytes) {
   if (workspace_bytes) *workspace_bytes = url_workspace_bytes(n_spans, arena_bytes, nfa_words);
   return layout_parts(url_layout(n_spans, arena_bytes, nfa_words, refs != 0), off, bytes, cap, end);
+}
+
+extern "C" void osehost_url_slices(uint32_t n_groups, uint32_t k, uint32_t form, uint32_t* out) {
+  if (k == 0) {
+    k = url_tail_slices(n_groups);
+    form = kUrlTailForm;
+  }
+  const UrlSlices S = url_slices(n_groups, k, form);
+  out[0] = S.k;
+  out[1] = size_partials_cap();
+  for (uint32_t j = 0; j <= kUrlMaxSlices; j++) {
+    out[2 + j] = S.g[j < S.k ? j : S.k];
+    out[3 + kUrlMaxSlices + j] = S.part[j < S.k ? j : S.k];
+  }
 }
 
 extern "C" int osehost_url_blob_hash(const char* cfg_json, int force_nfa, uint64_t* hash, uint64_t* bytes,
diff --git a/odigos_amd/csrc/url_kernel.hip b/odigos_amd/csrc/url_kernel.hip
--- a/odigos_amd/csrc/url_kernel.hip
+++ b/odigos_amd/csrc/url_kernel.hip
@@ -1298,8 +1298,8 @@
     a.dbg = nullptr;
   }
   const uint32_t stride = wave_stride();
-  uint32_t g = wave_first_group();
-  if (g >= a.n_groups) return;
+  uint32_t g = a.g_begin + wave_first_group();
+  if (g >= a.g_end) return;
   const bool tm = (kMode & kModeDiag) && a.dbg != nullptr;
   uint64_t t0 = 0, t_stage = 0, t_bm = 0, t_plan = 0, t_emit = 0, tt[3] = {0, 0, 0};
   const bool fused_cfg = sm.bn.ok && !(a.ablate & 2);
@@ -1327,7 +1327,7 @@
     lds_u32* stage32 = (lds_u32*)stage;
     const uint64_t i = (uint64_t)g * kWave + lane;
     const uint32_t g2 = g + stride;
-    const bool more = g2 < a.n_groups;
+    const bool more = g2 < a.g_end;
     const bool np2 = more && plan_gate(nxt) == 2;
     nn = plan_cols(a, (uint64_t)(g2 + stride) * kWave + lane);
     if (tm) { const uint64_t t1 = clk(); t_stage += t1 - t0; t0 = t1; }
@@ -1594,19 +1594,20 @@
   const uint32_t stride = wave_stride();
   uint32_t kept = 0;
   const bool sz_on = kSize && !sizedev::size_batch_dropped(a.sz);
-  uint32_t g = wave_first_group();
-  if (kRefs && !sz_on) g = a.n_groups;
+  const uint32_t g_end = kRefs ? a.g_end : a.n_groups;
+  uint32_t g = (kRefs ? a.g_begin : 0u) + wave_first_group();
+  if (kRefs && !sz_on) g = g_end;
   CopyCols An{0, 0, 0, ~0ull};
   sizedev::SpanCols xn{};
-  if (g < a.n_groups) {
+  if (g < g_end) {
     An = kRefs ? copy_len(a, g, lane) : copy_cols(a, g, lane);
     if (kSize && sz_on) xn = sizedev::size_span_load(a.sz, (uint64_t)g * kWave + lane, false);
   }
-  for (; g < a.n_groups; g += stride) {
+  for (; g < g_end; g += stride) {
     const uint64_t ia = (uint64_t)g * kWave + lane;
     const CopyCols A = An;
     const sizedev::SpanCols x0 = xn;
-    const bool more = g + stride < a.n_groups;
+    const bool more = g + stride < g_end;
     if (more) {
       An = kRefs ? copy_len(a, g + stride, lane) : copy_cols(a, g + stride, lane);
       if (kSize && sz_on) xn = sizedev::size_span_load(a.sz, (uint64_t)(g + stride) * kWave + lane, false);
@@ -1638,7 +1639,7 @@
     if (threadIdx.x == 0) {
       uint32_t t = 0;
       for (int w = 0; w < kWaves; w++) t += wk[w];
-      a.size_partials[blockIdx.x] = t;
+      a.size_partials[(kRefs ? a.partial_off : 0u) + blockIdx.x] = t;
     }
   }
 }
@@ -1652,6 +1653,7 @@
 __global__ __launch_bounds__(kWave) void url_plan_slow_kernel(UrlKernelArgs a) {
   __shared__ SlowPlanSmem sm;
   const uint32_t count = *a.unplanned_count;
+  if (a.unplanned_total && blockIdx.x == 0 && threadIdx.x == 0 && count) atomicAdd(a.unplanned_total, count);
   if (blockIdx.x >= count) return;
   const int lane = threadIdx.x;
   const uint64_t c0 = a.dbg ? clk() : 0;
@@ -1934,7 +1936,8 @@
   return (a.general ? kModeGeneral : 0) | ((OSE_DIAG && (a.ablate || a.dbg)) ? kModeDiag : 0);
 }
 template <int M>
-static uint32_t plan_blocks(const UrlKernelArgs& a) {
+static uint32_t plan_blocks(UrlKernelArgs a) {
+  a.n_groups = a.g_end - a.g_begin;
   static const uint32_t res = resident_blocks(url_plan_kernel<M>, 0);
   const uint32_t cap = a.refs && a.plan_grid_mult > 1 ? res * a.plan_grid_mult : std::min<uint32_t>(res, kUrlMaxWaves / kWaves);
   return std::min<uint32_t>(cap, (a.n_groups + kWaves - 1) / kWaves);
@@ -1973,7 +1976,7 @@
   return std::max<uint32_t>(1, std::min<uint32_t>(kUrlCopyMaxBlocks, (n_groups + 2 * kWaves - 1) / (2 * kWaves)));
 }
 void launch_url_copy(const UrlKernelArgs& a, hipStream_t st) {
-  const uint32_t blocks = url_copy_blocks(a.n_groups);
+  const uint32_t blocks = a.copy_blocks ? a.copy_blocks : url_copy_blocks(a.n_groups);
   if (a.refs) {
     if (a.fuse_size) hipLaunchKernelGGL((url_copy_kernel<true, true>), dim3(blocks), dim3(kThreads), 0, st, a);
   } else if (a.fuse_size) {
@@ -1991,7 +1994,7 @@
       per_cu = 2;
     return (uint32_t)(cus * per_cu);
   }();
-  const uint32_t blocks = std::min<uint32_t>(cap, a.n_groups);
+  const uint32_t blocks = std::min<uint32_t>(cap, a.g_end - a.g_begin);
   if (blocks) hipLaunchKernelGGL(url_plan_slow_kernel, dim3(blocks), dim3(kWave), 0, st, a);
 }
 void launch_url_emit_slow(const UrlKernelArgs& a, hipStream_t st) {
diff --git a/odigos_amd/native.py b/odigos_amd/native.py
--- a/odigos_amd/native.py
+++ b/odigos_amd/native.py
@@ -219,6 +219,7 @@
                                             C.POINTER(C.c_uint64)]),
         "osehost_stage_offsets": (None, [C.c_uint32, C.c_int, C.c_uint64, C.c_uint64, C.c_uint64, C.c_uint64, C.c_uint32,
                                          C.POINTER(C.c_uint64)]),
+        "osehost_url_slices": (None, [C.c_uint32, C.c_uint32, C.c_uint32, C.POINTER(C.c_uint32)]),
         "osehost_gbt_copy_times": (C.c_int, [_p, C.c_int, C.POINTER(C.c_double)]),
         "osehost_gbt_state": (C.c_int, [_p, C.POINTER(C.c_uint64), C.c_uint32]),
         "osehost_gbt_layout": (C.c_uint32, [C.c_uint32, C.c_uint64, C.c_uint64, C.c_uint64, C.c_uint64, C.c_uint32, C.c_int,
```

Result: faster. 14.97 billion spans/s (median of 6 runs) (+2.2%).
